# TangJiakai/RecBole-FairRec

Hardware: AMD Instinct MI355X
Metric: training interactions/sec + achieved HBM GB/s, FOCF emb=64 at 1/2/4/8 MI355X (higher is better)
Workload: dtype f32; 1 GPU; FOCF fair_objective=value, 1000001 users x 100001 items, embedding_size=64, B=8192 per GPU, Adam lr=1e-3 weight_decay=1e-3 (BASELINE.json configs[1]); ranks_seen=1, item_distribution=uniform, launch=hipGraph, lazy_adam_sweep_period=123, tables=single GPU, global_batch=8192, aged_steps=123

## Files before the change

### recbole-fairrec_amd/csrc/focf_step.hip

```cpp
#include <stddef.h>
#include <stdlib.h>

#include <algorithm>

#include "common.hpp"
#include "kernels.hpp"
#include "table.hpp"
#include "focf_ws.hpp"
#include "focf_loss.hpp"

namespace fr {

#ifndef FR_LPT_SHARED_FIRST
#define FR_LPT_SHARED_FIRST 1
#endif
#ifndef FR_STEP_WPB
#define FR_STEP_WPB 4
#endif
constexpr int STEP_WPB = FR_STEP_WPB;

struct StepArgs {
    float *Up, *Um, *Uv;
    int32_t *Ulast, *Ustamp;
    float *Ip, *Im, *Iv;
    int32_t *Ilast, *Istamp;
    int D, step;
    AdamC c;
    int B, objective;
    float fair_weight;
    const int4* task_rec;
    const int4* task_info;
    int lead;
    const int32_t* hdr;
    float* mse_e;
    float* term;
    void* ws;
    long long lo_u, lo_i;
    int n_u, n_i, skip_from;
    const int32_t* sw_order;
    uint32_t* err;
    unsigned long long *hcu, *hci;
    PrevLoss prev;
};

struct KV {
    unsigned v0, v1;
};
template <typename T>
__device__ __forceinline__ T karg(KV kv, int off) {
    static_assert(sizeof(T) == 4 || sizeof(T) == 8, "4- or 8-byte argument fields");
    const int d = off >> 2;
    auto word = [&](int i) { return (unsigned)__builtin_amdgcn_readlane((int)(i < 64 ? kv.v0 : kv.v1), i & 63); };
    if constexpr (sizeof(T) == 4) {
        return __builtin_bit_cast(T, word(d));
    } else {
        const unsigned long long q = (unsigned long long)word(d) | ((unsigned long long)word(d + 1) << 32);
        return __builtin_bit_cast(T, q);
    }
}
#define KA(field) karg<decltype(StepArgs::field)>(kv, (int)offsetof(StepArgs, field))
#define KAC(field) karg<decltype(AdamC::field)>(kv, (int)(offsetof(StepArgs, c) + offsetof(AdamC, field)))
static_assert(sizeof(StepArgs) <= 512, "the argument block must fit two VGPRs of dwords");

__device__ __forceinline__ int4 uload4(const int4* p, int idx) {
    const int4 v = p[idx];
    return make_int4(uniform(v.x), uniform(v.y), uniform(v.z), uniform(v.w));
}
__device__ __forceinline__ int uload(const int32_t* p, long long idx) { return uniform(p[idx]); }

__device__ __forceinline__ float ld_sc1(const float* p) {
    return __hip_atomic_load(p, __ATOMIC_RELAXED, __HIP_MEMORY_SCOPE_AGENT);
}
__device__ __forceinline__ void st_sc1(float* p, float v) {
    __hip_atomic_store(p, v, __ATOMIC_RELAXED, __HIP_MEMORY_SCOPE_AGENT);
}
__device__ __forceinline__ void drain_stores() { asm volatile("s_waitcnt vmcnt(0)" ::: "memory"); }

typedef __attribute__((address_space(1))) float gfloat;
typedef __attribute__((address_space(1))) int32_t gint;
__device__ __forceinline__ const gfloat* gp(const float* p) { return (const gfloat*)p; }
__device__ __forceinline__ gfloat* gp(float* p) { return (gfloat*)p; }
__device__ __forceinline__ const gint* gp(const int32_t* p) { return (const gint*)p; }
__device__ __forceinline__ gint* gp(int32_t* p) { return (gint*)p; }
typedef int v4i_ __attribute__((ext_vector_type(4)));
typedef __attribute__((address_space(1))) v4i_ gint4;
struct GInt4Ptr {
    const gint4* p;
    __device__ __forceinline__ int4 operator[](long long i) const {
        const v4i_ v = p[i];
        return make_int4(v.x, v.y, v.z, v.w);
    }
};
__device__ __forceinline__ GInt4Ptr gp(const int4* p) { return GInt4Ptr{(const gint4*)p}; }

__device__ __forceinline__ void st_sc1g(gfloat* p, float v) {
    __hip_atomic_store(p, v, __ATOMIC_RELAXED, __HIP_MEMORY_SCOPE_AGENT);
}

template <int E, bool FULL>
__device__ __forceinline__ void ldrow(RowFrag<E>& f, const float* base, int D, int lane) {
    const gfloat* g = gp(base);
#pragma unroll
    for (int e = 0; e < E; ++e) {
        const int d = lane + 64 * e;
        f.x[e] = (FULL || d < D) ? g[d] : 0.f;
    }
}

template <int E, bool FULL>
__device__ __forceinline__ void load_row_sc1(RowFrag<E>& f, const float* base, int D, int lane) {
    const gfloat* g = gp(base);
#pragma unroll
    for (int e = 0; e < E; ++e) {
        const int d = lane + 64 * e;
        f.x[e] = (FULL || d < D) ? __hip_atomic_load(g + d, __ATOMIC_RELAXED, __HIP_MEMORY_SCOPE_AGENT) : 0.f;
    }
}

template <int E, bool FULL>
__device__ __forceinline__ void store_row_sc1(const RowFrag<E>& f, float* base, int D, int lane) {
    gfloat* g = gp(base);
#pragma unroll
    for (int e = 0; e < E; ++e) {
        const int d = lane + 64 * e;
        float val = f.x[e];
        asm volatile("" : "+v"(val));
        if (FULL || d < D) st_sc1g(g + d, val);
    }
}

#ifndef FR_TROW_STORE
#define FR_TROW_STORE 1
#endif
#ifndef FR_WORD_STORE
#define FR_WORD_STORE 1
#endif
__device__ __forceinline__ void store_word(int32_t* p, int v) {
#if FR_TROW_STORE == 1 && FR_WORD_STORE
    __hip_atomic_store((gint*)p, v, __ATOMIC_RELAXED, __HIP_MEMORY_SCOPE_AGENT);
#else
    *(gint*)p = v;
#endif
}
__device__ __forceinline__ void store_word(float* p, float v) {
#if FR_TROW_STORE == 1 && FR_WORD_STORE
    st_sc1g((gfloat*)p, v);
#else
    *(gfloat*)p = v;
#endif
}

template <int E, bool FULL, bool WT = true>
__device__ __forceinline__ void store_trow(const RowFrag<E>& f, float* base, int D, int lane) {
    gfloat* g = gp(base);
#pragma unroll
    for (int e = 0; e < E; ++e) {
        const int d = lane + 64 * e;
#if FR_TROW_STORE == 1
        if (WT) {
            if (FULL || d < D) { float val = f.x[e]; asm volatile("" : "+v"(val)); st_sc1g(g + d, val); }
        } else if (FULL || d < D) g[d] = f.x[e];
#elif FR_TROW_STORE == 2
        if (WT) {
            if (FULL || d < D) __builtin_nontemporal_store(f.x[e], g + d);
        } else if (FULL || d < D) g[d] = f.x[e];
#else
        if (FULL || d < D) g[d] = f.x[e];
#endif
    }
}

constexpr int SW_NC = 16;
constexpr int HC_TAG_SHIFT = 29;
constexpr unsigned long long HC_CNT1 = 1ull << 14;
__device__ __forceinline__ int hc_base(unsigned long long w) { return (int)(w & 0x3fffull); }
__device__ __forceinline__ int hc_cnt(unsigned long long w) { return (int)((w >> 14) & 0x7fffull); }
static_assert(FR_SORT_MAX <= (1 << 14), "a batch's member list is addressed with 14 bits");

__device__ __forceinline__ unsigned ord_enc(float x) {
    const unsigned b = __float_as_uint(x);
    return (b & 0x80000000u) ? ~b : (b | 0x80000000u);
}
__device__ __forceinline__ float ord_dec(unsigned e) { return __uint_as_float((e & 0x80000000u) ? (e & 0x7fffffffu) : ~e); }

struct ClaimJob {
    const int64_t *user, *item;
    const float *rating, *sst;
    int4 *rec, *info;
    int32_t* cp;
    unsigned long long *hcu, *hci;
    int B, stamp;
    long long lo_u, lo_i;
    int n_u, n_i;
    int32_t* sw_tmp;
};
struct PlaceJob {
    int4 *rec, *info, *task_rec, *task_info;
    int32_t *cp, *hdr;
    unsigned long long *hcu, *hci;
    int B, n_pairs, stamp;
    const int32_t* sw_tmp;
    int32_t* sw_order;
};
struct StageArgs {
    ClaimJob c;
    PlaceJob p;
    int nb_claim, nb_sa, nb_place, nb_sb;
    int32_t *Ulast, *Ustamp, *Ilast, *Istamp;
    int n_rows_u, n_rows_i, cap;
    uint32_t* err;
};
constexpr int STAGE_THREADS = 64 * STEP_WPB;

template <int NC>
__device__ __forceinline__ int class_rank(int k, int32_t* counters, int lane) {
    const unsigned long long lt = (1ull << lane) - 1ull;
    unsigned long long m[NC];
    int mine = 0;
#pragma unroll
    for (int c = 0; c < NC; ++c) {
        m[c] = __ballot(k == c);
        if (lane == c) mine = __popcll(m[c]);
    }
    int got = 0;
    if (lane < NC && mine) got = atomicAdd(counters + lane, mine);
    int rk = 0;
#pragma unroll
    for (int c = 0; c < NC; ++c) {
        const int base = __shfl(got, c, 64);
        if (k == c) rk = base + __popcll(m[c] & lt);
    }
    return rk;
}

__device__ __forceinline__ int replay_class(int a, int b, int cap, int NC) {
    a = a < 0 ? 0 : (a > cap ? cap : a);
    b = b < 0 ? 0 : (b > cap ? cap : b);
    const int hi = a > b ? a : b, lo = a > b ? b : a;
    const int cost = 7 * hi + 2 * lo;
    return NC - 1 - min(NC - 1, cost * NC / (9 * cap + 1));
}

#ifndef FR_STAGE_EPT
#define FR_STAGE_EPT 2
#endif
constexpr int STAGE_EPT = FR_STAGE_EPT;
constexpr int STAGE_BLOCK = STAGE_THREADS * STAGE_EPT;

__device__ __forceinline__ void stage_claim(const StageArgs& s, int sb) {
    const ClaimJob& J = s.c;
    const int lane = threadIdx.x & 63;
    constexpr int EPT = STAGE_EPT;
    int b[EPT];
    bool ok[EPT];
    long long u[EPT], i[EPT];
    float rt[EPT], ss[EPT];
#pragma unroll
    for (int e = 0; e < EPT; ++e) {
        b[e] = (sb * EPT + e) * STAGE_THREADS + (int)threadIdx.x;
        ok[e] = b[e] < J.B;
        const int bc = ok[e] ? b[e] : 0;
        u[e] = J.user[bc];
        i[e] = J.item[bc];
        rt[e] = J.rating[bc];
        ss[e] = J.sst ? J.sst[bc] : 0.f;
    }
    bool bad = false;
#pragma unroll
    for (int e = 0; e < EPT; ++e) {
        bad |= ok[e] && (u[e] < 0 || u[e] >= s.n_rows_u || i[e] < 0 || i[e] >= s.n_rows_i);
        if (u[e] < 0 || u[e] >= s.n_rows_u) u[e] = 0;
        if (i[e] < 0 || i[e] >= s.n_rows_i) i[e] = 0;
    }
    if (bad && s.err) atomicOr(s.err, FR_DEV_ERR_INDEX_RANGE);
    const unsigned long long T = (unsigned long long)J.stamp << HC_TAG_SHIFT;
    unsigned long long mu[EPT], mi[EPT], ou[EPT], oi[EPT];
#pragma unroll
    for (int e = 0; e < EPT; ++e) {
        mu[e] = mi[e] = 0ull;
        if (ok[e]) {
            mu[e] = __hip_atomic_fetch_max(J.hcu + u[e], T, __ATOMIC_RELAXED, __HIP_MEMORY_SCOPE_AGENT);
            mi[e] = __hip_atomic_fetch_max(J.hci + i[e], T, __ATOMIC_RELAXED, __HIP_MEMORY_SCOPE_AGENT);
            atomicMax(s.Ustamp + u[e], J.stamp);
            atomicMax(s.Istamp + i[e], J.stamp);
        }
    }
#pragma unroll
    for (int e = 0; e < EPT; ++e) {
        ou[e] = oi[e] = 0ull;
        if (ok[e]) {
            ou[e] = __hip_atomic_fetch_add(J.hcu + u[e], HC_CNT1 + (mu[e] >> 63), __ATOMIC_RELAXED, __HIP_MEMORY_SCOPE_AGENT);
            oi[e] = __hip_atomic_fetch_add(J.hci + i[e], HC_CNT1 + (mi[e] >> 63), __ATOMIC_RELAXED, __HIP_MEMORY_SCOPE_AGENT);
        }
    }
    int first = 0;
    unsigned e1 = 0u, e2 = 0u;
#pragma unroll
    for (int e = 0; e < EPT; ++e) {
        const int ru = hc_cnt(ou[e]), ri = hc_cnt(oi[e]);
        if (ok[e]) {
            J.rec[b[e]] = make_int4((int)u[e], (int)i[e], __float_as_int(rt[e]), __float_as_int(ss[e]));
            J.info[b[e]] = make_int4(ru, ri, 0, 0);
            e1 = max(e1, ord_enc(ss[e]));
            e2 = max(e2, ord_enc(-ss[e]));
        }
        first += __popcll(__ballot(ok[e] && ri == 0));
    }
    if (lane == 0 && first) atomicAdd(J.cp + 8, first);
    if (J.sst) {
#pragma unroll
        for (int o = 32; o > 0; o >>= 1) {
            e1 = max(e1, (unsigned)__shfl_xor((int)e1, o, 64));
            e2 = max(e2, (unsigned)__shfl_xor((int)e2, o, 64));
        }
        if (lane == 0) {
            atomicMax(reinterpret_cast<unsigned*>(J.cp + 9), e1);
            atomicMax(reinterpret_cast<unsigned*>(J.cp + 10), e2);
        }
    }
}

__device__ __forceinline__ void stage_sweep_class(const StageArgs& s, int sb) {
    const ClaimJob& J = s.c;
    const int lane = threadIdx.x & 63;
    constexpr int EPT = STAGE_EPT;
    const int pairs_u = (J.n_u + 1) >> 1, n_pairs = pairs_u + ((J.n_i + 1) >> 1);
    const int cap = s.cap > 0 ? s.cap : 1024;
    int q[EPT], la[EPT], lb[EPT], sa[EPT], sb_[EPT], k[EPT];
#pragma unroll
    for (int e = 0; e < EPT; ++e) {
        q[e] = (sb * EPT + e) * STAGE_THREADS + (int)threadIdx.x;
        const int qc = q[e] < n_pairs ? q[e] : 0;
        const bool inU = qc < pairs_u;
        const int kk = inU ? qc : qc - pairs_u;
        const long long rowA = (inU ? J.lo_u : J.lo_i) + 2 * kk;
        const long long rowB = 2 * kk + 1 < (inU ? J.n_u : J.n_i) ? rowA + 1 : rowA;
        const int32_t* Tl = inU ? s.Ulast : s.Ilast;
        const int32_t* Ts = inU ? s.Ustamp : s.Istamp;
        la[e] = Tl[rowA]; lb[e] = Tl[rowB]; sa[e] = Ts[rowA]; sb_[e] = Ts[rowB];
    }
    int mine = 0;
#pragma unroll
    for (int e = 0; e < EPT; ++e) {
        k[e] = q[e] < n_pairs ? replay_class(sa[e] >= J.stamp ? 0 : J.stamp - la[e], sb_[e] >= J.stamp ? 0 : J.stamp - lb[e],
                                            cap, SW_NC)
                              : -1;
#pragma unroll
        for (int c = 0; c < SW_NC; ++c) {
            const int n = __popcll(__ballot(k[e] == c));
            if (lane == c) mine += n;
        }
    }
    int got = 0;
    if (lane < SW_NC && mine) got = atomicAdd(J.cp + 16 + lane, mine);
    const unsigned long long lt = (1ull << lane) - 1ull;
    int rk[EPT];
#pragma unroll
    for (int e = 0; e < EPT; ++e) rk[e] = 0;
#pragma unroll
    for (int c = 0; c < SW_NC; ++c) {
        int run = __shfl(got, c, 64);
#pragma unroll
        for (int e = 0; e < EPT; ++e) {
            const unsigned long long m = __ballot(k[e] == c);
            if (k[e] == c) rk[e] = run + __popcll(m & lt);
            run += __popcll(m);
        }
    }
#pragma unroll
    for (int e = 0; e < EPT; ++e)
        if (k[e] >= 0) J.sw_tmp[q[e]] = k[e] << 20 | rk[e];
}

#ifndef FR_PLACE_EPT
#define FR_PLACE_EPT 1
#endif
constexpr int PLACE_EPT = FR_PLACE_EPT;
__device__ __forceinline__ void stage_place(const StageArgs& s, int sb) {
    const PlaceJob& J = s.p;
    const int lane = threadIdx.x & 63;
    constexpr int EPT = PLACE_EPT;
    int b[EPT];
    bool ok[EPT];
    int4 rec[EPT], f[EPT];
#pragma unroll
    for (int e = 0; e < EPT; ++e) {
        b[e] = (sb * EPT + e) * STAGE_THREADS + (int)threadIdx.x;
        ok[e] = b[e] < J.B;
        const int bc = ok[e] ? b[e] : 0;
        rec[e] = J.rec[bc];
        f[e] = J.info[bc];
    }
    int nu[EPT], ni[EPT], k[EPT], key[EPT];
    {
        unsigned long long wu[EPT], wi[EPT];
        int lu[EPT], li[EPT];
#pragma unroll
        for (int e = 0; e < EPT; ++e) {
            wu[e] = J.hcu[rec[e].x];
            wi[e] = J.hci[rec[e].y];
            lu[e] = s.Ulast[rec[e].x];
            li[e] = s.Ilast[rec[e].y];
        }
        const int cap = s.cap > 0 ? s.cap : 1024;
#pragma unroll
        for (int e = 0; e < EPT; ++e) {
            nu[e] = hc_cnt(wu[e]);
            ni[e] = hc_cnt(wi[e]);
            if (ok[e] && nu[e] > 1 && f[e].x == 0) {
                const int base = atomicAdd(J.cp + 11, nu[e]);
                __hip_atomic_fetch_add(J.hcu + rec[e].x, (unsigned long long)base, __ATOMIC_RELAXED, __HIP_MEMORY_SCOPE_AGENT);
            }
            if (ok[e] && ni[e] > 1 && f[e].y == 0) {
                const int base = atomicAdd(J.cp + 12, ni[e]);
                __hip_atomic_fetch_add(J.hci + rec[e].y, (unsigned long long)base, __ATOMIC_RELAXED, __HIP_MEMORY_SCOPE_AGENT);
            }
            k[e] = !ok[e] ? -1 : ((nu[e] > 1 || ni[e] > 1) && FR_LPT_SHARED_FIRST ? 0 : 1);
            int cu = J.stamp - 1 - lu[e], ci = J.stamp - 1 - li[e];
            cu = cu < 0 ? 0 : (cu > cap ? cap : cu);
            ci = ci < 0 ? 0 : (ci > cap ? cap : ci);
            key[e] = 7 * (cu > ci ? cu : ci) + 2 * (cu > ci ? ci : cu);
        }
    }
    int before[EPT];
#pragma unroll
    for (int e = 0; e < EPT; ++e) before[e] = 0;
    int n0 = 0, n1 = 0;
#pragma unroll
    for (int e2 = 0; e2 < EPT; ++e2) {
        n0 += __popcll(__ballot(k[e2] == 0));
        n1 += __popcll(__ballot(k[e2] == 1));
        for (int t = 0; t < 64; ++t) {
            const int kt = __builtin_amdgcn_readlane(k[e2], t), ct = __builtin_amdgcn_readlane(key[e2], t);
#pragma unroll
            for (int e = 0; e < EPT; ++e)
                before[e] += (kt == k[e] && (ct > key[e] || (ct == key[e] && (e2 < e || (e2 == e && t < lane))))) ? 1 : 0;
        }
    }
    int got = 0;
    if (lane == 0 && n0) got = atomicAdd(J.cp, n0);
    if (lane == 1 && n1) got = atomicAdd(J.cp + 1, n1);
    const int base0 = __shfl(got, 0, 64), base1 = __shfl(got, 1, 64);
#pragma unroll
    for (int e = 0; e < EPT; ++e) {
        if (!ok[e]) continue;
        const int pos = k[e] == 0 ? base0 + before[e] : J.B - 1 - (base1 + (n1 - 1 - before[e]));
        J.task_rec[pos] = rec[e];
        J.task_info[pos] = make_int4(f[e].x | nu[e] << 16, f[e].y | ni[e] << 16, 0, b[e]);
        J.info[b[e]] = make_int4(f[e].x, f[e].y, nu[e], ni[e]);
    }
    if (sb == 0 && threadIdx.x == 0) {
        const unsigned e1 = (unsigned)J.cp[9], e2 = (unsigned)J.cp[10];
        *reinterpret_cast<int4*>(J.hdr) = make_int4(J.cp[8], 0, __float_as_int(-ord_dec(e2)), __float_as_int(ord_dec(e1)));
    }
}

__device__ __forceinline__ void stage_sweep_place(const StageArgs& s, int sb) {
    const PlaceJob& J = s.p;
    int cnt[SW_NC];
#pragma unroll
    for (int c = 0; c < SW_NC; ++c) cnt[c] = J.cp[16 + c];
    int v[STAGE_EPT];
#pragma unroll
    for (int e = 0; e < STAGE_EPT; ++e) {
        const int q = (sb * STAGE_EPT + e) * STAGE_THREADS + (int)threadIdx.x;
        v[e] = q < J.n_pairs ? J.sw_tmp[q] : -1;
    }
#pragma unroll
    for (int e = 0; e < STAGE_EPT; ++e) {
        const int q = (sb * STAGE_EPT + e) * STAGE_THREADS + (int)threadIdx.x;
        if (v[e] >= 0) {
            const int k = v[e] >> 20;
            int pos = v[e] & 0xfffff;
#pragma unroll
            for (int c = 0; c < SW_NC; ++c) pos += c < k ? cnt[c] : 0;
            J.sw_order[pos] = q;
        }
    }
    if (sb == 0 && threadIdx.x == 0) J.sw_order[J.n_pairs] = J.n_pairs;
}

__device__ __forceinline__ void stage_block(const StageArgs& s, int sb) {
    if (sb < s.nb_claim) return stage_claim(s, sb);
    sb -= s.nb_claim;
    if (sb < s.nb_sa) return stage_sweep_class(s, sb);
    sb -= s.nb_sa;
    if (sb < s.nb_place) return stage_place(s, sb);
    sb -= s.nb_place;
    if (sb < s.nb_sb) stage_sweep_place(s, sb);
}

__device__ __forceinline__ unsigned long long uniform64(unsigned long long x) {
    return (unsigned long long)(unsigned)uniform((int)(unsigned)x) | ((unsigned long long)(unsigned)uniform((int)(x >> 32)) << 32);
}
__device__ __forceinline__ int ld_sc1_int(const int32_t* p) {
    return __hip_atomic_load(p, __ATOMIC_RELAXED, __HIP_MEMORY_SCOPE_AGENT);
}
__device__ __forceinline__ void st_sc1_int(int32_t* p, int v) {
    __hip_atomic_store(p, v, __ATOMIC_RELAXED, __HIP_MEMORY_SCOPE_AGENT);
}
__device__ __forceinline__ unsigned long long hc_arrive(unsigned long long* p, int lane) {
    unsigned long long t = 0;
    if (lane == 0) t = __hip_atomic_fetch_add(p, 0ull - HC_CNT1, __ATOMIC_RELAXED, __HIP_MEMORY_SCOPE_AGENT);
    return uniform64(t);
}

struct Members {
    int reg;
    const int32_t* sorted;
    int n;
};
__device__ __forceinline__ Members load_members(const int32_t* list, int32_t* sorted, int base, int n, int lane) {
    Members m;
    m.n = n;
    m.reg = 0;
    m.sorted = sorted + base;
    if (n <= 64) {
        const int v = lane < n ? ld_sc1_int(list + base + lane) : 0x7fffffff;
        int rank = 0;
        for (int t = 0; t < n; ++t) rank += __builtin_amdgcn_readlane(v, t) < v ? 1 : 0;
        m.reg = __builtin_amdgcn_ds_permute(rank << 2, v);
        return m;
    }
    for (int jb = 0; jb < n; jb += 64) {
        const int v = jb + lane < n ? ld_sc1_int(list + base + jb + lane) : 0x7fffffff;
        int rank = 0;
        for (int jc = 0; jc < n; jc += 64) {
            const int x = jc + lane < n ? ld_sc1_int(list + base + jc + lane) : 0x7fffffff;
            const int cn = min(64, n - jc);
            for (int t = 0; t < cn; ++t) rank += __builtin_amdgcn_readlane(x, t) < v ? 1 : 0;
        }
        if (jb + lane < n) st_sc1_int(sorted + base + rank, v);
    }
    drain_stores();
    return m;
}
__device__ __forceinline__ int members_chunk(const Members& m, int jb, int lane) {
    if (m.n <= 64) return lane < m.n ? m.reg : 0;
    int idx = jb + lane;
    asm volatile("" : "+v"(idx));
    return idx < m.n ? ld_sc1_int(m.sorted + idx) : 0;
}

__device__ __forceinline__ bool arrive_last(unsigned int* cnt, int n, int lane) {
    unsigned t = 0;
    if (lane == 0) t = __hip_atomic_fetch_add(cnt, 1u, __ATOMIC_RELAXED, __HIP_MEMORY_SCOPE_AGENT);
    t = (unsigned)uniform((int)t);
    if (t != (unsigned)(n - 1)) return false;
    if (lane == 0) *cnt = 0u;
    return true;
}

template <int E, bool FULL>
__device__ __forceinline__ void adam_write(float* Tp, float* Tm, float* Tv, int32_t* Tlast, int D, int step,
                                           const AdamC& c, int row, RowFrag<E>& p, RowFrag<E>& m, RowFrag<E>& v,
                                           const RowFrag<E>& g, float2 s, int lane) {
#pragma unroll
    for (int e = 0; e < E; ++e) adam_elem(p.x[e], m.x[e], v.x[e], g.x[e], s.x, s.y, c);
    store_trow<E, FULL, false>(p, Tp + (size_t)row * D, D, lane);
    store_trow<E, FULL, false>(m, Tm + (size_t)row * D, D, lane);
    store_trow<E, FULL, false>(v, Tv + (size_t)row * D, D, lane);
    if (lane == 0) Tlast[row] = step;
}

template <int E, bool FULL, typename Chunk>
__device__ __forceinline__ void handed_grad_sum(RowFrag<E>& g, int n, Chunk chunk, const float* coef, const float* other,
                                                int D, int lane) {
#pragma unroll
    for (int e = 0; e < E; ++e) g.x[e] = 0.f;
    constexpr int UN = 2;
    for (int jb = 0; jb < n; jb += 64) {
        const int cnt = min(64, n - jb);
        int my_b = chunk(jb);
        float my_c = 0.f;
        if (lane >= cnt) my_b = 0;
        if (lane < cnt) my_c = ld_sc1(coef + my_b);
        for (int t0 = 0; t0 < cnt; t0 += UN) {
            RowFrag<E> o[UN];
            float cb[UN];
#pragma unroll
            for (int q = 0; q < UN; ++q) {
                const int t = t0 + q < cnt ? t0 + q : cnt - 1;
                const int b = __builtin_amdgcn_readlane(my_b, t);
                cb[q] = __builtin_bit_cast(float, __builtin_amdgcn_readlane(__builtin_bit_cast(int, my_c), t));
                load_row_sc1<E, FULL>(o[q], other + (size_t)b * D, D, lane);
            }
            {
#pragma clang fp contract(off)
#pragma unroll
                for (int q = 0; q < UN; ++q) {
                    if (t0 + q < cnt) {
#pragma unroll
                        for (int e = 0; e < E; ++e) {
                            float prod = cb[q] * o[q].x[e];
                            g.x[e] = g.x[e] + prod;
                        }
                    }
                }
            }
        }
    }
}

template <int E>
struct TwoRows {
    RowFrag<E> pA, mA, vA, pB, mB, vB;
};

template <int E>
__device__ __forceinline__ TwoRows<E> replay_two_v(TwoRows<E> r, int tA, int tB, int upto, const AdamC& c, int lane) {
    tA = tA < upto ? tA : upto;
    tB = tB < upto ? tB : upto;
    if (tA != tB) {
        const bool a_old = tA < tB;
        RowFrag<E> p, m, v;
#pragma unroll
        for (int e = 0; e < E; ++e) {
            p.x[e] = a_old ? r.pA.x[e] : r.pB.x[e];
            m.x[e] = a_old ? r.mA.x[e] : r.mB.x[e];
            v.x[e] = a_old ? r.vA.x[e] : r.vB.x[e];
        }
        replay<E>(p, m, v, a_old ? tA : tB, a_old ? tB : tA, c, lane);
#pragma unroll
        for (int e = 0; e < E; ++e) {
            if (a_old) {
                r.pA.x[e] = p.x[e]; r.mA.x[e] = m.x[e]; r.vA.x[e] = v.x[e];
            } else {
                r.pB.x[e] = p.x[e]; r.mB.x[e] = m.x[e]; r.vB.x[e] = v.x[e];
            }
        }
    }
    replay2<E>(r.pA, r.mA, r.vA, r.pB, r.mB, r.vB, tA > tB ? tA : tB, upto, c, lane);
    return r;
}
template <int E>
__device__ __forceinline__ void replay_two(TwoRows<E>& r, int tA, int tB, int upto, const AdamC& c, int lane) {
    r = replay_two_v<E>(r, tA, tB, upto, c, lane);
}

template <int E, bool FULL>
__device__ __forceinline__ void user_finish(KV kv, const AdamC& c, const FocfWs& w, int j0u, int nu, float2 s, int lane) {
    const int D = FULL ? 64 * E : KA(D);
    const int c0 = uniform(w.perm_u[j0u]);
    const int ur = uniform(w.rec[c0].x);
    RowFrag<E> p, m, v, g;
    load_row_sc1<E, FULL>(p, w.side[0] + (size_t)c0 * D, D, lane);
    load_row_sc1<E, FULL>(m, w.side[1] + (size_t)c0 * D, D, lane);
    load_row_sc1<E, FULL>(v, w.side[2] + (size_t)c0 * D, D, lane);
    handed_grad_sum<E, FULL>(g, nu, [&](int jb) { return jb + lane < nu ? w.perm_u[j0u + jb + lane] : 0; }, w.coef, w.side[3],
                             D, lane);
    adam_write<E, FULL>(KA(Up), KA(Um), KA(Uv), KA(Ulast), D, KA(step), c, ur, p, m, v, g, s, lane);
}

template <int E, bool FULL>
__device__ __forceinline__ void user_finish_c(KV kv, const AdamC& c, const FocfWs& w, int ur, int base, int nu, float2 s,
                                              int lane) {
    const int D = FULL ? 64 * E : KA(D);
    const Members mem = load_members(w.perm_u, w.seg_start_u, base, nu, lane);
    const int c0 = __builtin_amdgcn_readlane(members_chunk(mem, 0, lane), 0);
    RowFrag<E> p, m, v, g;
    load_row_sc1<E, FULL>(p, w.side[0] + (size_t)c0 * D, D, lane);
    load_row_sc1<E, FULL>(m, w.side[1] + (size_t)c0 * D, D, lane);
    load_row_sc1<E, FULL>(v, w.side[2] + (size_t)c0 * D, D, lane);
    handed_grad_sum<E, FULL>(g, nu, [&](int jb) { return members_chunk(mem, jb, lane); }, w.coef, w.side[3], D, lane);
    adam_write<E, FULL>(KA(Up), KA(Um), KA(Uv), KA(Ulast), D, KA(step), c, ur, p, m, v, g, s, lane);
}

template <int E, bool FULL, bool CLAIM>
__device__ __forceinline__ void step_shared_rows(KV kv, const AdamC& c, int b, int lane, int ur, int ir, int iux, int iix,
                                                 int seg_u, int seg_i, float dot, float coef, float smin, float smax,
                                                 float K, RowFrag<E>& pu, RowFrag<E>& mu, RowFrag<E>& vu, RowFrag<E>& pi,
                                                 RowFrag<E>& mi, RowFrag<E>& vi) {
    const int D = FULL ? 64 * E : KA(D);
    const bool fair = KA(objective) != FR_FOCF_NONE;
    const int nu = iux >> 16, ni = iix >> 16, j0u = iux & 0xffff, j0i = iix & 0xffff;
    const float2 s = step_scalars(c, KA(step));
    int Bq = KA(B);
    asm volatile("" : "+s"(Bq));
    const FocfWs w = focf_layout(KA(ws), Bq, D);

    if constexpr (CLAIM) {
        unsigned long long wu = 0, wi = 0;
        if (nu > 1) wu = __hip_atomic_load(KA(hcu) + ur, __ATOMIC_RELAXED, __HIP_MEMORY_SCOPE_AGENT);
        if (ni > 1) wi = __hip_atomic_load(KA(hci) + ir, __ATOMIC_RELAXED, __HIP_MEMORY_SCOPE_AGENT);
        if (lane == 0) {
            if (nu > 1) st_sc1_int(w.perm_u + hc_base(wu) + j0u, b);
            if (ni > 1) st_sc1_int(w.perm_i + hc_base(wi) + j0i, b);
        }
    }
    const size_t so = (size_t)b * D;
    store_row_sc1<E, FULL>(pu, w.side[0] + so, D, lane);
    store_row_sc1<E, FULL>(mu, w.side[1] + so, D, lane);
    store_row_sc1<E, FULL>(vu, w.side[2] + so, D, lane);
    if (nu > 1) store_row_sc1<E, FULL>(pi, w.side[3] + so, D, lane);
    if (ni == 1) {
        RowFrag<E> gi;
#pragma unroll
        for (int e = 0; e < E; ++e) gi.x[e] = coef * pu.x[e];
        adam_write<E, FULL>(KA(Ip), KA(Im), KA(Iv), KA(Ilast), D, KA(step), c, ir, pi, mi, vi, gi, s, lane);
        if (lane == 0) st_sc1(w.coef + b, coef);
        drain_stores();
        if constexpr (CLAIM) {
            const unsigned long long old = hc_arrive(KA(hcu) + ur, lane);
            if (hc_cnt(old) == 1) user_finish_c<E, FULL>(kv, c, w, ur, hc_base(old), nu, s, lane);
        } else {
            if (arrive_last(w.cnt_u + seg_u, nu, lane)) user_finish<E, FULL>(kv, c, w, j0u, nu, s, lane);
        }
        return;
    }
    if (lane == 0) {
        st_sc1(w.pred + b, dot);
        if (CLAIM && fair) st_sc1(w.term + b, 0.f);
    }
    drain_stores();
    Members mem{};
    if constexpr (CLAIM) {
        const unsigned long long old = hc_arrive(KA(hci) + ir, lane);
        if (hc_cnt(old) != 1) return;
        mem = load_members(w.perm_i, w.seg_start_i, hc_base(old), ni, lane);
    } else {
        if (!arrive_last(w.cnt_i + seg_i, ni, lane)) return;
    }

    const bool big = ni > 64;
    int my_b = 0, my_u = 0, my_iux = 0, my_seg = 0;
    float my_pr = 0.f, my_rt = 0.f, my_s = 0.f;
    auto load_chunk = [&](int jb) {
        my_b = 0; my_u = 0; my_iux = 0; my_seg = 0;
        my_pr = 0.f; my_rt = 0.f; my_s = 0.f;
        int mb = 0;
        if constexpr (CLAIM) mb = members_chunk(mem, jb, lane);
        if (jb + lane < ni) {
            if constexpr (CLAIM) my_b = mb;
            else my_b = w.perm_i[j0i + jb + lane];
            const int4 rq = w.rec[my_b];
            const int4 fq = w.info[my_b];
            my_pr = ld_sc1(w.pred + my_b);
            my_u = rq.x; my_rt = __int_as_float(rq.z); my_s = __int_as_float(rq.w);
            if constexpr (CLAIM) {
                my_iux = fq.z << 16;
            } else {
                my_iux = fq.x; my_seg = fq.y;
            }
        }
    };
    float term = 0.f, g0 = 0.f, g1 = 0.f;
    if (fair) {
        float sp0 = 0.f, sp1 = 0.f, st0 = 0.f, st1 = 0.f, n0 = 0.f, n1 = 0.f;
        bool bad = false;
        int first_b = 0;
        for (int jb = 0; jb < ni; jb += 64) {
            load_chunk(jb);
            if (jb == 0) first_b = __builtin_amdgcn_readlane(my_b, 0);
#pragma unroll
            for (int k = 0; k < 64 / FAIR_GROUP; ++k) {
                const int src = (lane & (FAIR_GROUP - 1)) + FAIR_GROUP * k;
                const float pr = __shfl(my_pr, src, 64), rr = __shfl(my_rt, src, 64), sq = __shfl(my_s, src, 64);
                if (lane < FAIR_GROUP && jb + src < ni) {
                    bad |= (sq != smin && sq != smax);
                    if (sq == smin) {
                        sp0 += pr; st0 += rr; n0 += 1.f;
                    } else {
                        sp1 += pr; st1 += rr; n1 += 1.f;
                    }
                }
            }
        }
        if (bad && KA(err)) atomicOr(KA(err), FR_DEV_ERR_SST_GROUPS);
        sp0 = group_sum<FAIR_GROUP>(sp0); sp1 = group_sum<FAIR_GROUP>(sp1);
        st0 = group_sum<FAIR_GROUP>(st0); st1 = group_sum<FAIR_GROUP>(st1);
        n0 = group_sum<FAIR_GROUP>(n0);   n1 = group_sum<FAIR_GROUP>(n1);
        sp0 = __builtin_bit_cast(float, uniform(__builtin_bit_cast(int, sp0)));
        sp1 = __builtin_bit_cast(float, uniform(__builtin_bit_cast(int, sp1)));
        st0 = __builtin_bit_cast(float, uniform(__builtin_bit_cast(int, st0)));
        st1 = __builtin_bit_cast(float, uniform(__builtin_bit_cast(int, st1)));
        n0 = __builtin_bit_cast(float, uniform(__builtin_bit_cast(int, n0)));
        n1 = __builtin_bit_cast(float, uniform(__builtin_bit_cast(int, n1)));
        focf_fair_eval(KA(objective), KA(fair_weight), K, sp0, sp1, st0, st1, n0, n1, term, g0, g1);
        if (lane == 0) KA(term)[CLAIM ? first_b : seg_i] = term;
    }
    constexpr int UN = E == 1 ? 4 : (E == 2 ? 2 : 1);
    RowFrag<E> gi;
#pragma unroll
    for (int e = 0; e < E; ++e) gi.x[e] = 0.f;
    bool shared_users = false;
    for (int jb = 0; jb < ni; jb += 64) {
        if (big || !fair) load_chunk(jb);
        const int cnt = min(64, ni - jb);
        float my_c = 0.f;
        if (lane < cnt) {
            const float erq = my_pr - my_rt;
            my_c = 2.f * erq / (float)KA(B);
            if (fair) my_c = my_c + (my_s == smin ? g0 : g1);
            if ((my_iux >> 16) > 1) st_sc1(w.coef + my_b, my_c);
        }
        shared_users |= __ballot(lane < cnt && (my_iux >> 16) > 1) != 0ull;
        for (int t0 = 0; t0 < cnt; t0 += UN) {
            RowFrag<E> p[UN], m[UN], v[UN];
            int uq[UN], nq[UN];
            float cq[UN];
#pragma unroll
            for (int q = 0; q < UN; ++q) {
                const int t = t0 + q < cnt ? t0 + q : cnt - 1;
                const int bq = __builtin_amdgcn_readlane(my_b, t);
                uq[q] = __builtin_amdgcn_readlane(my_u, t);
                nq[q] = __builtin_amdgcn_readlane(my_iux, t) >> 16;
                cq[q] = __builtin_bit_cast(float, __builtin_amdgcn_readlane(__builtin_bit_cast(int, my_c), t));
                const size_t sq = (size_t)bq * D;
                load_row_sc1<E, FULL>(p[q], w.side[0] + sq, D, lane);
                load_row_sc1<E, FULL>(m[q], w.side[1] + sq, D, lane);
                load_row_sc1<E, FULL>(v[q], w.side[2] + sq, D, lane);
            }
#pragma unroll
            for (int q = 0; q < UN; ++q) {
                if (t0 + q >= cnt) continue;
                {
#pragma clang fp contract(off)
#pragma unroll
                    for (int e = 0; e < E; ++e) {
                        float prod = cq[q] * p[q].x[e];
                        gi.x[e] = gi.x[e] + prod;
                    }
                }
                if (nq[q] == 1) {
                    RowFrag<E> gu;
#pragma unroll
                    for (int e = 0; e < E; ++e) gu.x[e] = cq[q] * pi.x[e];
                    adam_write<E, FULL>(KA(Up), KA(Um), KA(Uv), KA(Ulast), D, KA(step), c, uq[q], p[q], m[q], v[q], gu, s, lane);
                }
            }
        }
    }
    adam_write<E, FULL>(KA(Ip), KA(Im), KA(Iv), KA(Ilast), D, KA(step), c, ir, pi, mi, vi, gi, s, lane);
    if (!shared_users) return;
    drain_stores();
    for (int jb = 0; jb < ni; jb += 64) {
        if (big) load_chunk(jb);
        const int cnt = min(64, ni - jb);
        unsigned long long todo = __ballot(lane < cnt && (my_iux >> 16) > 1);
        while (todo) {
            const int t = __builtin_ctzll(todo);
            todo &= todo - 1;
            const int iq = __builtin_amdgcn_readlane(my_iux, t);
            if constexpr (CLAIM) {
                const int uu = __builtin_amdgcn_readlane(my_u, t);
                const unsigned long long old = hc_arrive(KA(hcu) + uu, lane);
                if (hc_cnt(old) == 1) user_finish_c<E, FULL>(kv, c, w, uu, hc_base(old), iq >> 16, s, lane);
            } else {
                const int sg = __builtin_amdgcn_readlane(my_seg, t);
                if (arrive_last(w.cnt_u + sg, iq >> 16, lane)) user_finish<E, FULL>(kv, c, w, iq & 0xffff, iq >> 16, s, lane);
            }
        }
    }
}

__device__ __forceinline__ void focf_fair_single(int objective, float fair_weight, float K, bool in0, float pred,
                                                 float rating, float& term, float& g) {
    const float cc = 1.f + 1e-5f;
    const float P = pred / cc, T = rating / cc;
    float d, q;
    if (objective == FR_FOCF_VALUE) {
        d = P - T; q = 1.f;
    } else if (objective == FR_FOCF_ABSOLUTE) {
        d = fabsf(P - T); q = (P > T) ? 1.f : (P < T ? -1.f : 0.f);
    } else if (objective == FR_FOCF_UNDER) {
        d = (T - P > 0.f) ? T - P : 0.f; q = (T - P > 0.f) ? -1.f : 0.f;
    } else {
        d = (P - T > 0.f) ? P - T : 0.f; q = (P - T > 0.f) ? 1.f : 0.f;
    }
    const float delta = in0 ? d - 0.f : 0.f - d;
    const float x = fabsf(delta);
    term = smooth_l1(x);
    const float sgn = delta > 0.f ? 1.f : (delta < 0.f ? -1.f : 0.f);
    const float dx = (x < 1.f ? x : 1.f) * sgn * fair_weight / K;
    g = in0 ? dx * q / cc : -dx * q / cc;
}

template <int E, bool FULL, bool CLAIM>
__device__ __forceinline__ void step_finish(KV kv, const AdamC& c, int lane, int q, RowFrag<E>& pu, RowFrag<E>& mu,
                                            RowFrag<E>& vu, RowFrag<E>& pi, RowFrag<E>& mi, RowFrag<E>& vi) {
    const int D = FULL ? 64 * E : KA(D);
    const bool fair = KA(objective) != FR_FOCF_NONE;
    const int4 vrec = KA(task_rec)[q], vinf = KA(task_info)[q], vhd = *reinterpret_cast<const int4*>(KA(hdr));
    const int4 rec = make_int4(uniform(vrec.x), uniform(vrec.y), uniform(vrec.z), uniform(vrec.w));
    const int4 inf = make_int4(uniform(vinf.x), uniform(vinf.y), uniform(vinf.z), uniform(vinf.w));
    const int4 hd = make_int4(uniform(vhd.x), 0, uniform(vhd.z), uniform(vhd.w));
    const int ur = rec.x, ir = rec.y;
    const float rt = __int_as_float(rec.z), s = __int_as_float(rec.w);
    const int iux = inf.x, iix = inf.y, b = inf.w;
    const float K = (float)hd.x, smin = __int_as_float(hd.z), smax = __int_as_float(hd.w);
    const int nu = iux >> 16, ni = iix >> 16, seg_u = inf.z & 0xffff, seg_i = inf.z >> 16;
    float dot = 0.f;
#pragma unroll
    for (int e = 0; e < E; ++e) dot = fmaf(pu.x[e], pi.x[e], dot);
    dot = wave_sum(dot);
    const float er = dot - rt;
    if (lane == 0) store_word(KA(mse_e) + b, er * er);
    const float cm = 2.f * er / (float)KA(B);
    float coef = cm;
    if (ni == 1 && fair) {
        const bool in0 = s == smin;
        if (s != smin && s != smax && lane == 0 && KA(err)) atomicOr(KA(err), FR_DEV_ERR_SST_GROUPS);
        float term, g;
        focf_fair_single(KA(objective), KA(fair_weight), K, in0, dot, rt, term, g);
        coef = cm + g;
        if (lane == 0) KA(term)[CLAIM ? b : seg_i] = term;
    }
    if (ni == 1 && nu == 1) {
        const float2 sc = step_scalars(c, KA(step));
#pragma unroll
        for (int e = 0; e < E; ++e) {
            v2f_ P = {pu.x[e], pi.x[e]}, M = {mu.x[e], mi.x[e]}, V = {vu.x[e], vi.x[e]};
            const v2f_ G = __builtin_elementwise_fma(v2f_{c.wd, c.wd}, P, v2f_{coef * P.y, coef * P.x});
            M = __builtin_elementwise_fma(v2f_{c.omb1, c.omb1}, G - M, M);
            V = __builtin_elementwise_fma(G * c.omb2, G, V * c.b2);
            const v2f_ den = __builtin_elementwise_fma(v2f_{__builtin_amdgcn_sqrtf(V.x), __builtin_amdgcn_sqrtf(V.y)},
                                                      v2f_{sc.y, sc.y}, v2f_{c.eps, c.eps});
            P = __builtin_elementwise_fma(M * -sc.x, v2f_{__builtin_amdgcn_rcpf(den.x), __builtin_amdgcn_rcpf(den.y)}, P);
            pu.x[e] = P.x; pi.x[e] = P.y;
            mu.x[e] = M.x; mi.x[e] = M.y;
            vu.x[e] = V.x; vi.x[e] = V.y;
        }
        store_trow<E, FULL>(pu, KA(Up) + (size_t)ur * D, D, lane);
        store_trow<E, FULL>(mu, KA(Um) + (size_t)ur * D, D, lane);
        store_trow<E, FULL>(vu, KA(Uv) + (size_t)ur * D, D, lane);
        store_trow<E, FULL>(pi, KA(Ip) + (size_t)ir * D, D, lane);
        store_trow<E, FULL>(mi, KA(Im) + (size_t)ir * D, D, lane);
        store_trow<E, FULL>(vi, KA(Iv) + (size_t)ir * D, D, lane);
        if (lane == 0) {
            store_word(KA(Ulast) + ur, KA(step));
            store_word(KA(Ilast) + ir, KA(step));
        }
        return;
    }
    step_shared_rows<E, FULL, CLAIM>(kv, c, b, lane, ur, ir, iux, iix, seg_u, seg_i, dot, coef, smin, smax, K, pu, mu, vu, pi, mi,
                                     vi);
}

template <int E, bool FULL>
__device__ __forceinline__ void adam_store_both(KV kv, const AdamC& c, int lane, int ur, int ir, float coef, float2 sc,
                                                RowFrag<E> pu, RowFrag<E> mu, RowFrag<E> vu, RowFrag<E> pi,
                                                RowFrag<E> mi, RowFrag<E> vi) {
    const int D = FULL ? 64 * E : KA(D);
#pragma unroll
    for (int e = 0; e < E; ++e) {
        v2f_ P = {pu.x[e], pi.x[e]}, M = {mu.x[e], mi.x[e]}, V = {vu.x[e], vi.x[e]};
        const v2f_ G = __builtin_elementwise_fma(v2f_{c.wd, c.wd}, P, v2f_{coef * P.y, coef * P.x});
        M = __builtin_elementwise_fma(v2f_{c.omb1, c.omb1}, G - M, M);
        V = __builtin_elementwise_fma(G * c.omb2, G, V * c.b2);
        const v2f_ den = __builtin_elementwise_fma(v2f_{__builtin_amdgcn_sqrtf(V.x), __builtin_amdgcn_sqrtf(V.y)},
                                                  v2f_{sc.y, sc.y}, v2f_{c.eps, c.eps});
        P = __builtin_elementwise_fma(M * -sc.x, v2f_{__builtin_amdgcn_rcpf(den.x), __builtin_amdgcn_rcpf(den.y)}, P);
        pu.x[e] = P.x; pi.x[e] = P.y;
        mu.x[e] = M.x; mi.x[e] = M.y;
        vu.x[e] = V.x; vi.x[e] = V.y;
    }
    store_trow<E, FULL>(pu, KA(Up) + (size_t)ur * D, D, lane);
    store_trow<E, FULL>(mu, KA(Um) + (size_t)ur * D, D, lane);
    store_trow<E, FULL>(vu, KA(Uv) + (size_t)ur * D, D, lane);
    store_trow<E, FULL>(pi, KA(Ip) + (size_t)ir * D, D, lane);
    store_trow<E, FULL>(mi, KA(Im) + (size_t)ir * D, D, lane);
    store_trow<E, FULL>(vi, KA(Iv) + (size_t)ir * D, D, lane);
    if (lane == 0) {
        store_word(KA(Ulast) + ur, KA(step));
        store_word(KA(Ilast) + ir, KA(step));
    }
}

template <int E, bool FULL, bool CLAIM>
__device__ __forceinline__ void step_finish_pair(KV kv, const AdamC& c, int lane, int q, int q1, bool has1, TwoRows<E> us,
                                                 TwoRows<E> is) {
    const int obj = KA(objective);
    const bool fair = obj != FR_FOCF_NONE;
    const GInt4Ptr trec = gp(KA(task_rec));
    const GInt4Ptr tinf = gp(KA(task_info));
    const int4 vr0 = trec[q], vr1 = trec[q1], vi0 = tinf[q], vi1 = tinf[q1];
    const int4 vhd = gp(reinterpret_cast<const int4*>(KA(hdr)))[0];
    float d0 = 0.f, d1 = 0.f;
#pragma unroll
    for (int e = 0; e < E; ++e) {
        d0 = fmaf(us.pA.x[e], is.pA.x[e], d0);
        d1 = fmaf(us.pB.x[e], is.pB.x[e], d1);
    }
#pragma unroll
    for (int o = 32; o > 0; o >>= 1) {
        const float y0 = __shfl_xor(d0, o, 64), y1 = __shfl_xor(d1, o, 64);
        d0 += y0;
        d1 += y1;
    }
    const bool odd = (lane & 1) != 0;
    const int rec_z = odd ? vr1.z : vr0.z, rec_w = odd ? vr1.w : vr0.w;
    const int inf_y = odd ? vi1.y : vi0.y, inf_z = odd ? vi1.z : vi0.z, inf_w = odd ? vi1.w : vi0.w;
    const float dot = odd ? d1 : d0;
    const float rt = __int_as_float(rec_z), sst = __int_as_float(rec_w);
    const float K = (float)vhd.x, smin = __int_as_float(vhd.z), smax = __int_as_float(vhd.w);
    const int ni_l = inf_y >> 16;
    const float er = dot - rt;
    const float cm = 2.f * er / (float)KA(B);
    float coef = cm, term = 0.f;
    const bool single = fair && ni_l == 1;
    if (fair) {
        float g;
        focf_fair_single(obj, KA(fair_weight), K, sst == smin, dot, rt, term, g);
        if (single) coef = cm + g;
    }
    if (lane < (has1 ? 2 : 1)) {
        store_word(KA(mse_e) + inf_w, er * er);
        if (single) {
            store_word(KA(term) + (CLAIM ? inf_w : inf_z >> 16), term);
            if (sst != smin && sst != smax && KA(err)) atomicOr(KA(err), FR_DEV_ERR_SST_GROUPS);
        }
    }
    const float coef0 = __builtin_bit_cast(float, __builtin_amdgcn_readlane(__builtin_bit_cast(int, coef), 0));
    const float coef1 = __builtin_bit_cast(float, __builtin_amdgcn_readlane(__builtin_bit_cast(int, coef), 1));
    const int ur0 = uniform(vr0.x), ir0 = uniform(vr0.y), ur1 = uniform(vr1.x), ir1 = uniform(vr1.y);
    const int iux0 = uniform(vi0.x), iix0 = uniform(vi0.y), iux1 = uniform(vi1.x), iix1 = uniform(vi1.y);
    const bool un0 = (iux0 >> 16) == 1 && (iix0 >> 16) == 1;
    const bool un1 = has1 && (iux1 >> 16) == 1 && (iix1 >> 16) == 1;
    const float2 sc = step_scalars(c, KA(step));
    if (un0 && un1) {
        RowFrag<E> a0 = us.pA, a1 = us.mA, a2 = us.vA, a3 = is.pA, a4 = is.mA, a5 = is.vA;
        RowFrag<E> b0 = us.pB, b1 = us.mB, b2 = us.vB, b3 = is.pB, b4 = is.mB, b5 = is.vB;
        adam_store_both<E, FULL>(kv, c, lane, ur0, ir0, coef0, sc, a0, a1, a2, a3, a4, a5);
        adam_store_both<E, FULL>(kv, c, lane, ur1, ir1, coef1, sc, b0, b1, b2, b3, b4, b5);
        return;
    }
    if (un0) adam_store_both<E, FULL>(kv, c, lane, ur0, ir0, coef0, sc, us.pA, us.mA, us.vA, is.pA, is.mA, is.vA);
    if (un1) adam_store_both<E, FULL>(kv, c, lane, ur1, ir1, coef1, sc, us.pB, us.mB, us.vB, is.pB, is.mB, is.vB);
    if (un0 && (un1 || !has1)) return;
    for (int k = 0; k < (has1 ? 2 : 1); ++k) {
        if (k) {
#pragma unroll
            for (int e = 0; e < E; ++e) {
                us.pA.x[e] = us.pB.x[e]; us.mA.x[e] = us.mB.x[e]; us.vA.x[e] = us.vB.x[e];
                is.pA.x[e] = is.pB.x[e]; is.mA.x[e] = is.mB.x[e]; is.vA.x[e] = is.vB.x[e];
            }
        }
        if (!(k ? un1 : un0)) {
            const int sg = uniform(k ? vi1.z : vi0.z);
            step_shared_rows<E, FULL, CLAIM>(kv, c, uniform(k ? vi1.w : vi0.w), lane, k ? ur1 : ur0, k ? ir1 : ir0, k ? iux1 : iux0,
                                      k ? iix1 : iix0, sg & 0xffff, sg >> 16, k ? d1 : d0, k ? coef1 : coef0, smin, smax, K,
                                      us.pA, us.mA, us.vA, is.pA, is.mA, is.vA);
        }
    }
}

#if FR_STEP_TRACE
#define g_phase phase_stamps
#endif
template <int E, bool FULL, bool PAIR, bool CLAIM>
__device__ __forceinline__ void step_task(KV kv, bool sweeper, int q, int n_pairs, int lane, const int4* rec0,
                                          const int32_t* order0, int B0
#if FR_STEP_TRACE
                                          , unsigned long long (&phase_stamps)[4]
#endif
) {
    asm volatile("" : "+v"(lane));
    AdamC c;
    c.sc = KAC(sc); c.cap = KAC(cap); c.wd = KAC(wd); c.b1 = KAC(b1); c.omb1 = KAC(omb1); c.b2 = KAC(b2); c.omb2 = KAC(omb2);
    c.eps = KAC(eps); c.k1 = KAC(k1); c.k2 = KAC(k2); c.inv_k1 = KAC(inv_k1); c.inv_k2 = KAC(inv_k2);
    const int D = FULL ? 64 * E : KA(D);
    TwoRows<E> r;
    int tA, tB;
    if (sweeper) {
        if (const int32_t* so = order0) {
            const int oq = so[q], on = so[n_pairs];
            q = uniform(on) == n_pairs ? uniform(oq) : q;
        }
        const int pairs_u = (KA(n_u) + 1) >> 1;
        const bool inU = q < pairs_u;
        const int k = inU ? q : q - pairs_u;
        const long long rowA = (inU ? KA(lo_u) : KA(lo_i)) + 2 * k;
        const bool hasB = 2 * k + 1 < (inU ? KA(n_u) : KA(n_i));
        const long long rowB = hasB ? rowA + 1 : rowA;
        float* Tp = inU ? KA(Up) : KA(Ip);
        float* Tm = inU ? KA(Um) : KA(Im);
        float* Tv = inU ? KA(Uv) : KA(Iv);
        int32_t* Tl = inU ? KA(Ulast) : KA(Ilast);
        const int32_t* Ts = inU ? KA(Ustamp) : KA(Istamp);
        const int sa = gp(Ts)[rowA], sb = gp(Ts)[rowB];
        const int la = gp((const int32_t*)Tl)[rowA], lb = gp((const int32_t*)Tl)[rowB];
        ldrow<E, FULL>(r.pA, Tp + (size_t)rowA * D, D, lane);
        ldrow<E, FULL>(r.mA, Tm + (size_t)rowA * D, D, lane);
        ldrow<E, FULL>(r.vA, Tv + (size_t)rowA * D, D, lane);
        ldrow<E, FULL>(r.pB, Tp + (size_t)rowB * D, D, lane);
        ldrow<E, FULL>(r.mB, Tm + (size_t)rowB * D, D, lane);
        ldrow<E, FULL>(r.vB, Tv + (size_t)rowB * D, D, lane);
        const int upto = KA(step);
        tA = uniform(sa) >= KA(skip_from) ? upto : uniform(la);
        tB = (!hasB || uniform(sb) >= KA(skip_from)) ? upto : uniform(lb);
        const bool doA = tA < upto, doB = tB < upto;
        replay_two<E>(r, tA, tB, upto, c, lane);
        if (doA) {
            store_trow<E, FULL>(r.pA, Tp + (size_t)rowA * D, D, lane);
            store_trow<E, FULL>(r.mA, Tm + (size_t)rowA * D, D, lane);
            store_trow<E, FULL>(r.vA, Tv + (size_t)rowA * D, D, lane);
            if (lane == 0) store_word(Tl + rowA, upto);
        }
        if (doB) {
            store_trow<E, FULL>(r.pB, Tp + (size_t)rowB * D, D, lane);
            store_trow<E, FULL>(r.mB, Tm + (size_t)rowB * D, D, lane);
            store_trow<E, FULL>(r.vB, Tv + (size_t)rowB * D, D, lane);
            if (lane == 0) store_word(Tl + rowB, upto);
        }
        return;
    }
    if (PAIR) {
        const bool has1 = q + 1 < B0;
        const int q1 = has1 ? q + 1 : q;
        const int4 vrec0 = gp(rec0)[q], vrec1 = gp(rec0)[q1];
        const int u0 = uniform(vrec0.x), i0 = uniform(vrec0.y), u1 = uniform(vrec1.x), i1 = uniform(vrec1.y);
#if FR_STEP_TRACE
        g_phase[2] = __builtin_amdgcn_s_memrealtime();
#endif
        const int lu0 = gp((const int32_t*)KA(Ulast))[u0], lu1 = gp((const int32_t*)KA(Ulast))[u1];
        const int li0 = gp((const int32_t*)KA(Ilast))[i0], li1 = gp((const int32_t*)KA(Ilast))[i1];
        TwoRows<E> it;
        ldrow<E, FULL>(r.pA, KA(Up) + (size_t)u0 * D, D, lane);
        ldrow<E, FULL>(r.pB, KA(Up) + (size_t)u1 * D, D, lane);
        ldrow<E, FULL>(it.pA, KA(Ip) + (size_t)i0 * D, D, lane);
        ldrow<E, FULL>(it.pB, KA(Ip) + (size_t)i1 * D, D, lane);
        ldrow<E, FULL>(r.mA, KA(Um) + (size_t)u0 * D, D, lane);
        ldrow<E, FULL>(r.vA, KA(Uv) + (size_t)u0 * D, D, lane);
        ldrow<E, FULL>(r.mB, KA(Um) + (size_t)u1 * D, D, lane);
        ldrow<E, FULL>(r.vB, KA(Uv) + (size_t)u1 * D, D, lane);
        ldrow<E, FULL>(it.mA, KA(Im) + (size_t)i0 * D, D, lane);
        ldrow<E, FULL>(it.vA, KA(Iv) + (size_t)i0 * D, D, lane);
        ldrow<E, FULL>(it.mB, KA(Im) + (size_t)i1 * D, D, lane);
        ldrow<E, FULL>(it.vB, KA(Iv) + (size_t)i1 * D, D, lane);
        const int upto = KA(step) - 1;
        const int tu0 = uniform(lu0), tu1 = uniform(lu1), ti0 = uniform(li0), ti1 = uniform(li1);
#if FR_STEP_TRACE
        g_phase[0] = __builtin_amdgcn_s_memrealtime();
        g_phase[3] = (unsigned long long)((upto - tu0) + (upto - tu1) + (upto - ti0) + (upto - ti1));
#endif
        replay_two<E>(r, tu0, tu1, upto, c, lane);
        replay_two<E>(it, ti0, ti1, upto, c, lane);
#if FR_STEP_TRACE
        g_phase[1] = __builtin_amdgcn_s_memrealtime();
#endif
        step_finish_pair<E, FULL, CLAIM>(kv, c, lane, q, q1, has1, r, it);
        return;
    }
    const int4 vrec = rec0[q];
    const int ur = uniform(vrec.x), ir = uniform(vrec.y);
    const int lu = KA(Ulast)[ur], li = KA(Ilast)[ir];
    ldrow<E, FULL>(r.pA, KA(Up) + (size_t)ur * D, D, lane);
    ldrow<E, FULL>(r.pB, KA(Ip) + (size_t)ir * D, D, lane);
    ldrow<E, FULL>(r.mA, KA(Um) + (size_t)ur * D, D, lane);
    ldrow<E, FULL>(r.vA, KA(Uv) + (size_t)ur * D, D, lane);
    ldrow<E, FULL>(r.mB, KA(Im) + (size_t)ir * D, D, lane);
    ldrow<E, FULL>(r.vB, KA(Iv) + (size_t)ir * D, D, lane);
    tA = uniform(lu);
    tB = uniform(li);
    replay_two<E>(r, tA, tB, KA(step) - 1, c, lane);
    step_finish<E, FULL, CLAIM>(kv, c, lane, q, r.pA, r.mA, r.vA, r.pB, r.mB, r.vB);
}

__host__ __device__ constexpr bool step_pairs(int E) { return E <= 1; }

#ifndef FR_STEP_TRACE
#define FR_STEP_TRACE 0
#endif

#if FR_STEP_TRACE
__device__ unsigned long long g_step_trace[8 * 65536];
__device__ int g_trace_step = -1;
#endif

#ifndef FR_STEP_WAVES
#define FR_STEP_WAVES 6
#endif
__host__ __device__ constexpr int step_waves(int E) { return E >= 4 ? (FR_STEP_WAVES < 5 ? FR_STEP_WAVES : 5) : FR_STEP_WAVES; }
constexpr int STEP_PRELOAD_DWORDS = 10;
template <int E, bool FULL, bool CLAIM>
__global__ __launch_bounds__(64 * STEP_WPB, step_waves(E)) void focf_step_kernel(const int4* pre_rec, const int32_t* pre_order,
                                                                                 int pre_B, int pre_lead, int pre_nu, int pre_ni,
                                                                                 int pre_stage, int pre_pad, StepArgs a,
                                                                                 StageArgs st) {
#if FR_STEP_TRACE
    const unsigned long long tr0 = __builtin_amdgcn_s_memrealtime();
    const unsigned long long mt0 = __builtin_amdgcn_s_memtime();
    unsigned long long ph[4] = {0, 0, 0, 0};
#endif
    const int lane = threadIdx.x & 63;
    const int wib = uniform((int)(threadIdx.x >> 6));
    int role = 0;
    const int n_stage = CLAIM ? pre_stage : 0;
    (void)pre_pad;
#ifndef FR_STAGE_POS
#define FR_STAGE_POS 2
#endif
    const int stage0 = FR_STAGE_POS == 0 ? 1 : (FR_STAGE_POS == 1 ? (int)gridDim.x - n_stage : 1 + pre_lead);
    if (blockIdx.x == 0) {
        if (a.prev.loss_out) step_reduce_loss<64 * STEP_WPB>(a.prev);
    } else if (CLAIM && (int)blockIdx.x >= stage0 && (int)blockIdx.x < stage0 + n_stage) {
        if constexpr (CLAIM) stage_block(st, (int)blockIdx.x - stage0);
        role = 3;
    } else {
        const unsigned* kp = reinterpret_cast<const unsigned*>(
            (const void*)(const __attribute__((address_space(4))) void*)__builtin_amdgcn_kernarg_segment_ptr());
        KV kv;
        static_assert(STEP_PRELOAD_DWORDS * 4 % alignof(StepArgs) == 0, "StepArgs follows the preloaded scalars without padding");
        kv.v0 = kp[STEP_PRELOAD_DWORDS + lane];
        kv.v1 = lane < (int)(sizeof(StepArgs) / 4) - 64 ? kp[STEP_PRELOAD_DWORDS + 64 + lane] : 0u;
        const int x = (int)blockIdx.x - 1 - ((int)blockIdx.x >= stage0 ? n_stage : 0);
        const int n_pairs = ((pre_nu + 1) >> 1) + ((pre_ni + 1) >> 1);
        const int n_sweep = n_pairs;
        const int ns = (n_sweep + STEP_WPB - 1) / STEP_WPB;
        constexpr bool PAIR = step_pairs(E);
        const bool sweeper = x >= pre_lead && x < pre_lead + ns;
        const int q = ((sweeper ? x - pre_lead : (x < pre_lead ? x : x - ns)) * STEP_WPB + wib) * (!sweeper && PAIR ? 2 : 1);
        role = sweeper ? 1 : 2;
#if FR_STEP_TRACE
        if (q < (sweeper ? n_sweep : pre_B)) step_task<E, FULL, PAIR, CLAIM>(kv, sweeper, q, n_pairs, lane, pre_rec, pre_order, pre_B, ph);
#else
        if (q < (sweeper ? n_sweep : pre_B)) step_task<E, FULL, PAIR, CLAIM>(kv, sweeper, q, n_pairs, lane, pre_rec, pre_order, pre_B);
#endif
    }
#if FR_STEP_TRACE
    asm volatile("s_waitcnt vmcnt(0)" ::: "memory");
    const unsigned long long tr1 = __builtin_amdgcn_s_memrealtime();
    const unsigned long long mt1 = __builtin_amdgcn_s_memtime();
    unsigned hw, xcc;
    asm volatile("s_getreg_b32 %0, hwreg(HW_REG_HW_ID)" : "=s"(hw));
    asm volatile("s_getreg_b32 %0, hwreg(HW_REG_XCC_ID)" : "=s"(xcc));
    const int tsel = g_trace_step < 0 ? 0 : a.step - g_trace_step;
    const unsigned wq = blockIdx.x * STEP_WPB + wib + (g_trace_step < 0 ? 0u : 16384u * (unsigned)(tsel & 3));
    if (lane == 0 && wq < 65536 && (g_trace_step < 0 || (tsel >= 0 && tsel < 4 && blockIdx.x * STEP_WPB + wib < 16384))) {
        g_step_trace[4 * wq] = tr0;
        g_step_trace[4 * wq + 1] = tr1;
        g_step_trace[4 * wq + 2] = role;
        g_step_trace[4 * wq + 3] = (unsigned long long)hw | ((unsigned long long)xcc << 32);
        g_step_trace[4 * (65536 + wq)] = (ph[2] ? ((ph[2] - tr0) << 40) : 0ull) | (mt1 - mt0);
        g_step_trace[4 * (65536 + wq) + 1] = ph[0];
        g_step_trace[4 * (65536 + wq) + 2] = ph[1];
        g_step_trace[4 * (65536 + wq) + 3] = ph[3];
    }
#endif
}

__global__ __launch_bounds__(256) void focf_step_finish_kernel(PrevLoss pl) { step_reduce_loss<256>(pl); }

__global__ __launch_bounds__(STAGE_THREADS) void focf_stage_kernel(StageArgs st) { stage_block(st, (int)blockIdx.x); }

struct SwOrderJob {
    const int32_t *Ulast, *Ustamp, *Ilast, *Istamp;
    long long lo_u, lo_i;
    int n_u, n_i, upto, skip_from;
    int32_t* order;
};

template <int PT>
__device__ __forceinline__ void sweep_order_body(const SwOrderJob& J, int cap_, int* cnt, int* wsum) {
    constexpr int NC = SW_NC, NW = 16, N = NC * PT * NW, EPT = (N + 1023) / 1024;
    const int tid = threadIdx.x, lane = tid & 63, wave = tid >> 6;
    const unsigned long long lt = (1ull << lane) - 1ull;
    const int cap = cap_ > 0 ? cap_ : 1024;
    const int pairs_u = (J.n_u + 1) >> 1, n_pairs = pairs_u + ((J.n_i + 1) >> 1);
    if (!J.order) return;
    if (n_pairs > PT * 1024) {
        if (tid == 0 && n_pairs <= SWEEP_ORDER_MAX) J.order[n_pairs] = -1;
        return;
    }
    int la[PT], lb[PT], sa[PT], sb[PT];
#pragma unroll
    for (int r = 0; r < PT; ++r) {
        const int q = r * 1024 + tid, qc = q < n_pairs ? q : 0;
        const bool inU = qc < pairs_u;
        const int k = inU ? qc : qc - pairs_u;
        const long long rowA = (inU ? J.lo_u : J.lo_i) + 2 * k;
        const long long rowB = 2 * k + 1 < (inU ? J.n_u : J.n_i) ? rowA + 1 : rowA;
        const int32_t* Tl = inU ? J.Ulast : J.Ilast;
        const int32_t* Ts = inU ? J.Ustamp : J.Istamp;
        la[r] = Tl[rowA]; lb[r] = Tl[rowB]; sa[r] = Ts[rowA]; sb[r] = Ts[rowB];
    }
    int cls[PT], rank[PT];
#pragma unroll
    for (int r = 0; r < PT; ++r) {
        const int q = r * 1024 + tid;
        int k = -1;
        if (q < n_pairs) {
            int ca = sa[r] >= J.skip_from ? 0 : J.upto - la[r], cb = sb[r] >= J.skip_from ? 0 : J.upto - lb[r];
            ca = ca < 0 ? 0 : (ca > cap ? cap : ca);
            cb = cb < 0 ? 0 : (cb > cap ? cap : cb);
            const int hi = ca > cb ? ca : cb, lo = ca > cb ? cb : ca;
            const int cost = 7 * hi + 2 * lo;
            k = NC - 1 - min(NC - 1, cost * NC / (9 * cap + 1));
        }
        cls[r] = k;
        rank[r] = 0;
#pragma unroll
        for (int c = 0; c < NC; ++c) {
            const unsigned long long m = __ballot(k == c);
            if (k == c) rank[r] = __popcll(m & lt);
            if (lane == 0) cnt[(c * PT + r) * NW + wave] = __popcll(m);
        }
    }
    __syncthreads();
    {
        int x[EPT], own = 0;
#pragma unroll
        for (int e = 0; e < EPT; ++e) {
            const int i = tid * EPT + e;
            x[e] = i < N ? cnt[i] : 0;
            own += x[e];
        }
        int inc = own;
#pragma unroll
        for (int o = 1; o < 64; o <<= 1) {
            const int y = __shfl_up(inc, o, 64);
            if (lane >= o) inc += y;
        }
        if (lane == 63) wsum[wave] = inc;
        __syncthreads();
        int ex = inc - own;
        for (int w = 0; w < wave; ++w) ex += wsum[w];
#pragma unroll
        for (int e = 0; e < EPT; ++e) {
            const int i = tid * EPT + e;
            if (i < N) cnt[i] = ex;
            ex += x[e];
        }
    }
    __syncthreads();
#pragma unroll
    for (int r = 0; r < PT; ++r)
        if (cls[r] >= 0) J.order[cnt[(cls[r] * PT + r) * NW + wave] + rank[r]] = r * 1024 + tid;
    if (tid == 0) J.order[n_pairs] = n_pairs;
}

struct LptJob {
    const int32_t *age_u, *age_i;
    const int4 *rec, *info;
    int4 *task_rec, *task_info;
    int B, upto;
};
struct LptJobs {
    LptJob j[FR_FOCF_PREPARE_MAX];
    SwOrderJob sw[FR_FOCF_PREPARE_MAX];
    int n;
    int cap;
};

#ifdef FR_LPT_STAMPS
__device__ unsigned long long g_lpt_stamps[8];
#define LPT_STAMP(i) do { if (blockIdx.x == 0 && threadIdx.x == 0) g_lpt_stamps[i] = __builtin_amdgcn_s_memtime(); } while (0)
#else
#define LPT_STAMP(i) do {} while (0)
#endif

constexpr int LPT_SPLIT = 4;

template <int PT>
__global__ __launch_bounds__(1024) void focf_lpt_kernel(LptJobs jobs) {
    constexpr int NC = 8, NW = 16, N = NC * PT * NW, EPT = (N + 1023) / 1024;
    __shared__ int cnt[SW_NC * PT * NW];
    __shared__ int wsum[NW];
    if ((int)blockIdx.x >= jobs.n * LPT_SPLIT) {
        sweep_order_body<PT>(jobs.sw[blockIdx.x - jobs.n * LPT_SPLIT], jobs.cap, cnt, wsum);
        return;
    }
    const LptJob& J = jobs.j[blockIdx.x / LPT_SPLIT];
    const int part = blockIdx.x % LPT_SPLIT;
    const int tid = threadIdx.x, lane = tid & 63, wave = tid >> 6;
    const unsigned long long lt = (1ull << lane) - 1ull;
    const int cap = jobs.cap > 0 ? jobs.cap : 1024;
    int cls[PT], rank[PT];
    int lu[PT], li[PT];
    bool sh[PT];
    LPT_STAMP(0);
#pragma unroll
    for (int q = 0; q < PT; ++q) {
        const int b = q * 1024 + tid, bc = b < J.B ? b : 0;
        lu[q] = J.age_u[bc];
        li[q] = J.age_i[bc];
#if FR_LPT_SHARED_FIRST
        const int4 f = J.info[bc];
        sh[q] = (f.x >> 16) > 1 || (f.z >> 16) > 1;
#else
        sh[q] = false;
#endif
    }
    LPT_STAMP(1);
#pragma unroll
    for (int q = 0; q < PT; ++q) {
        const int b = q * 1024 + tid;
        int k = -1;
        if (b < J.B) {
            int cu = J.upto - lu[q], ci = J.upto - li[q];
            cu = cu < 0 ? 0 : (cu > cap ? cap : cu);
            ci = ci < 0 ? 0 : (ci > cap ? cap : ci);
            const int hi = cu > ci ? cu : ci, lo = cu > ci ? ci : cu;
            const int cost = 7 * hi + 2 * lo;
            k = NC - 1 - min(NC - 1, cost * NC / (9 * cap + 1));
            if (sh[q]) k = 0;
        }
        cls[q] = k;
        rank[q] = 0;
#pragma unroll
        for (int c = 0; c < NC; ++c) {
            const unsigned long long m = __ballot(k == c);
            if (k == c) rank[q] = __popcll(m & lt);
            if (lane == 0) cnt[(c * PT + q) * NW + wave] = __popcll(m);
        }
    }
    LPT_STAMP(2);
    __syncthreads();
    {
        int x[EPT], own = 0;
#pragma unroll
        for (int e = 0; e < EPT; ++e) {
            const int i = tid * EPT + e;
            x[e] = i < N ? cnt[i] : 0;
            own += x[e];
        }
        int inc = own;
#pragma unroll
        for (int o = 1; o < 64; o <<= 1) {
            const int y = __shfl_up(inc, o, 64);
            if (lane >= o) inc += y;
        }
        if (lane == 63) wsum[wave] = inc;
        __syncthreads();
        int ex = inc - own;
        for (int w = 0; w < wave; ++w) ex += wsum[w];
#pragma unroll
        for (int e = 0; e < EPT; ++e) {
            const int i = tid * EPT + e;
            if (i < N) cnt[i] = ex;
            ex += x[e];
        }
    }
    __syncthreads();
    LPT_STAMP(3);
    constexpr int CH = (PT + LPT_SPLIT - 1) / LPT_SPLIT;
    int4 f[CH], r[CH];
#pragma unroll
    for (int q = 0; q < CH; ++q) {
        const int b = (q * LPT_SPLIT + part) * 1024 + tid, bc = b < J.B ? b : 0;
        f[q] = J.info[bc];
        r[q] = J.rec[bc];
    }
#pragma unroll
    for (int q = 0; q < CH; ++q) {
#pragma unroll
        for (int pp = 0; pp < LPT_SPLIT; ++pp) {
            const int qq = q * LPT_SPLIT + pp;
            if (pp == part && qq < PT && cls[qq] >= 0) {
                const int pos = cnt[(cls[qq] * PT + qq) * NW + wave] + rank[qq];
                J.task_rec[pos] = r[q];
                J.task_info[pos] = make_int4(f[q].x, f[q].z, f[q].y | (f[q].w << 16), qq * 1024 + tid);
            }
        }
    }
    LPT_STAMP(4);
}

}

using namespace fr;

extern "C" int fr_focf_prepare_step(const fr_focf_batch* batches, const int32_t* stamps, int32_t n, const fr_table* U,
                                    const fr_table* I, int32_t replay_cap, uint32_t* err_flag, void* stream_) {
    int rc;
    if ((rc = check_table(U, "fr_focf_prepare_step(U)")) || (rc = check_table(I, "fr_focf_prepare_step(I)"))) return rc;
    FR_CHECK_ARG(batches && stamps && n >= 1 && 2 * n <= FR_SORT_JOBS && U->dim == I->dim,
                 "fr_focf_prepare_step: 1..%d batches", FR_SORT_JOBS / 2);
    SortJobList jobs{};
    for (int q = 0; q < n; ++q) {
        const fr_focf_batch& b = batches[q];
        FR_CHECK_ARG(b.user && b.item && b.rating && b.ws && b.B >= 1 && b.B <= FR_SORT_MAX,
                     "fr_focf_prepare_step: batch %d", q);
        FocfWs w = focf_layout(b.ws, b.B, U->dim);
        FR_CHECK_ARG(b.ws_bytes >= w.bytes, "fr_focf_prepare_step: workspace %zu < %zu bytes", b.ws_bytes, w.bytes);
        SortJob ju{b.user, U->n_rows, w.perm_u, w.seg_start_u, w.seg_row_u, nullptr, w.nseg_u, nullptr, nullptr};
        SortJob ji{b.item, I->n_rows, w.perm_i, w.seg_start_i, w.seg_row_i, nullptr, w.nseg_i, b.sst, w.sst_minmax};
        ju.seg_first = w.seg_first_u;
        ji.seg_first = w.seg_first_i;
        ju.info = reinterpret_cast<int2*>(w.info);
        ji.info = reinterpret_cast<int2*>(w.info) + 1;
        ju.info_stride = ji.info_stride = 2;
        ji.rec = w.rec;
        ji.rec_idx = b.user;
        ji.rec_rows = U->n_rows;
        ji.rec_f0 = b.rating;
        ju.cnt = w.cnt_u;
        ji.cnt = w.cnt_i;
        ju.stamp = U->stamp;
        ji.stamp = I->stamp;
        ju.stamp_val = ji.stamp_val = stamps[q];
        ju.last = U->last;
        ji.last = I->last;
        ju.last_out = w.age_u;
        ji.last_out = w.age_i;
        ji.pos_of = w.pos_i;
        jobs.j[2 * q] = ju;
        jobs.j[2 * q + 1] = ji;
        jobs.M[2 * q] = jobs.M[2 * q + 1] = (int)b.B;
    }
    jobs.n = 2 * n;
    if ((rc = launch_sort_many(jobs, U->n_rows > I->n_rows ? U->n_rows : I->n_rows, err_flag, (hipStream_t)stream_)))
        return rc;
    LptJobs lj{};
    for (int q = 0; q < n; ++q) {
        const FocfWs w = focf_layout(batches[q].ws, batches[q].B, U->dim);
        lj.j[q] = LptJob{w.age_u, w.age_i, w.rec, w.info, w.task_rec, w.task_info, (int)batches[q].B, stamps[q] - 1};
    }
    lj.cap = replay_cap;
    lj.n = n;
    for (int q = 0; q < n; ++q) {
        const FocfWs w = focf_layout(batches[q].ws, batches[q].B, U->dim);
        fr_table tu = *U, ti = *I;
        tu.step = ti.step = stamps[q];
        const SweepSlice sw = make_sweep_slice(&tu, &ti, replay_cap);
        lj.sw[q] = SwOrderJob{U->last, U->stamp, I->last, I->stamp, sw.lo_u, sw.lo_i, sw.n_u, sw.n_i, stamps[q], stamps[q],
                              replay_cap > 0 ? w.sw_order : nullptr};
    }
    int Bmax = 1;
    for (int q = 0; q < n; ++q) Bmax = batches[q].B > Bmax ? (int)batches[q].B : Bmax;
    hipStream_t st = (hipStream_t)stream_;
    ProfScope prof(K_FOCF_LPT, st);
    if (Bmax <= 1024) FR_LAUNCH(prof, focf_lpt_kernel<1>, dim3(n * (LPT_SPLIT + 1)), dim3(1024), 0, st, lj);
    else if (Bmax <= 2048) FR_LAUNCH(prof, focf_lpt_kernel<2>, dim3(n * (LPT_SPLIT + 1)), dim3(1024), 0, st, lj);
    else if (Bmax <= 4096) FR_LAUNCH(prof, focf_lpt_kernel<4>, dim3(n * (LPT_SPLIT + 1)), dim3(1024), 0, st, lj);
    else if (Bmax <= 8192) FR_LAUNCH(prof, focf_lpt_kernel<8>, dim3(n * (LPT_SPLIT + 1)), dim3(1024), 0, st, lj);
    else FR_LAUNCH(prof, focf_lpt_kernel<16>, dim3(n * (LPT_SPLIT + 1)), dim3(1024), 0, st, lj);
    FR_CHECK_LAUNCH();
    return FR_OK;
}

static unsigned long long* words_of(uint64_t* row_words, int32_t gen, const fr_table* U, const fr_table* I, bool item) {
    const size_t per = (size_t)U->n_rows + (size_t)I->n_rows;
    return reinterpret_cast<unsigned long long*>(row_words) + (size_t)gen * per + (item ? (size_t)U->n_rows : 0);
}

static int make_stages(StageArgs& st, const fr_table* U, const fr_table* I, const fr_focf_batch* claim, int32_t claim_stamp,
                       int32_t claim_gen, const fr_focf_batch* place, int32_t place_stamp, int32_t place_gen,
                       int32_t sweep_period, uint64_t* row_words, uint32_t* err_flag, int32_t claim_step, int32_t place_step) {
    if (claim_step < 1) claim_step = claim_stamp;
    if (place_step < 1) place_step = place_stamp;
    st = StageArgs{};
    st.Ulast = U->last; st.Ustamp = U->stamp; st.Ilast = I->last; st.Istamp = I->stamp;
    st.n_rows_u = (int)U->n_rows; st.n_rows_i = (int)I->n_rows;
    st.cap = sweep_period;
    st.err = err_flag;
    FR_CHECK_ARG(row_words && U->n_rows <= INT32_MAX && I->n_rows <= INT32_MAX, "fr_focf_stage: row words missing");
    FR_CHECK_ARG(U->stamp && I->stamp && U->last && I->last, "fr_focf_stage: the tables need their last / stamp arrays");
    auto slice_of = [&](int32_t step) {
        fr_table tu = *U, ti = *I;
        tu.step = ti.step = step;
        return make_sweep_slice(&tu, &ti, sweep_period);
    };
    if (claim) {
        const fr_focf_batch& b = *claim;
        FR_CHECK_ARG(b.user && b.item && b.rating && b.ws && b.B >= 1 && b.B <= FR_SORT_MAX && claim_stamp >= 1 &&
                         claim_gen >= 0 && claim_gen < 3, "fr_focf_stage: batch to claim");
        const FocfWs w = focf_layout(b.ws, b.B, U->dim);
        FR_CHECK_ARG(b.ws_bytes >= w.bytes, "fr_focf_stage: workspace %zu < %zu bytes", b.ws_bytes, w.bytes);
        ClaimJob& J = st.c;
        J.user = b.user; J.item = b.item; J.rating = b.rating; J.sst = b.sst;
        J.rec = w.rec; J.info = w.info; J.cp = w.cp;
        J.hcu = words_of(row_words, claim_gen, U, I, false);
        J.hci = words_of(row_words, claim_gen, U, I, true);
        J.B = (int)b.B; J.stamp = claim_stamp;
        st.nb_claim = (int)((b.B + STAGE_BLOCK - 1) / STAGE_BLOCK);
        if (sweep_period > 0) {
            const SweepSlice sw = slice_of(claim_step);
            const long long n_pairs = ((long long)sw.n_u + 1) / 2 + ((long long)sw.n_i + 1) / 2;
            if (n_pairs <= SWEEP_ORDER_MAX) {
                J.lo_u = sw.lo_u; J.lo_i = sw.lo_i; J.n_u = sw.n_u; J.n_i = sw.n_i;
                J.sw_tmp = w.sw_tmp;
                st.nb_sa = (int)((n_pairs + STAGE_BLOCK - 1) / STAGE_BLOCK);
            }
        }
    }
    if (place) {
        const fr_focf_batch& b = *place;
        FR_CHECK_ARG(b.ws && b.B >= 1 && b.B <= FR_SORT_MAX && place_stamp >= 1 && place_gen >= 0 && place_gen < 3,
                     "fr_focf_stage: batch to place");
        const FocfWs w = focf_layout(b.ws, b.B, U->dim);
        FR_CHECK_ARG(b.ws_bytes >= w.bytes, "fr_focf_stage: workspace %zu < %zu bytes", b.ws_bytes, w.bytes);
        PlaceJob& J = st.p;
        J.rec = w.rec; J.info = w.info; J.task_rec = w.task_rec; J.task_info = w.task_info;
        J.cp = w.cp; J.hdr = w.nseg_i;
        J.hcu = words_of(row_words, place_gen, U, I, false);
        J.hci = words_of(row_words, place_gen, U, I, true);
        J.B = (int)b.B; J.stamp = place_stamp;
        st.nb_place = (int)((b.B + STAGE_THREADS * PLACE_EPT - 1) / (STAGE_THREADS * PLACE_EPT));
        if (sweep_period > 0) {
            const SweepSlice sw = slice_of(place_step);
            const long long n_pairs = ((long long)sw.n_u + 1) / 2 + ((long long)sw.n_i + 1) / 2;
            if (n_pairs <= SWEEP_ORDER_MAX) {
                J.n_pairs = (int)n_pairs;
                J.sw_tmp = w.sw_tmp; J.sw_order = w.sw_order;
                st.nb_sb = (int)((n_pairs + STAGE_BLOCK - 1) / STAGE_BLOCK);
            }
        }
    }
    return FR_OK;
}

extern "C" size_t fr_focf_row_words(int64_t n_users, int64_t n_items) { return 3 * ((size_t)n_users + (size_t)n_items); }

extern "C" int fr_focf_stage(const fr_table* U, const fr_table* I, const fr_focf_batch* claim, int32_t claim_stamp,
                             int32_t claim_gen, const fr_focf_batch* place, int32_t place_stamp, int32_t place_gen,
                             int32_t sweep_period, uint64_t* row_words, uint32_t* err_flag, void* stream_) {
    int rc;
    if ((rc = check_table(U, "fr_focf_stage(U)")) || (rc = check_table(I, "fr_focf_stage(I)"))) return rc;
    FR_CHECK_ARG(U->dim == I->dim && (claim || place), "fr_focf_stage: nothing to do");
    StageArgs st;
    if ((rc = make_stages(st, U, I, claim, claim_stamp, claim_gen, place, place_stamp, place_gen, sweep_period, row_words,
                          err_flag, place ? U->step + 1 : U->step, U->step)))
        return rc;
    const int nb = st.nb_claim + st.nb_sa + st.nb_place + st.nb_sb;
    ProfScope prof(K_FOCF_STAGE, (hipStream_t)stream_);
    FR_LAUNCH(prof, focf_stage_kernel, dim3(nb), dim3(STAGE_THREADS), 0, (hipStream_t)stream_, st);
    FR_CHECK_LAUNCH();
    return FR_OK;
}

static int focf_step_impl(const fr_table* U, const fr_table* I, const fr_adam* adam, const float* sst, int64_t B,
                          int32_t objective, float fair_weight, int32_t sweep_period, int32_t stamp, void* ws,
                          size_t ws_bytes, void* prev_ws, int64_t prev_B, float* prev_loss_out, float* loss_acc,
                          uint32_t* err_flag, void* stream_, const StageArgs* stages, uint64_t* row_words, int32_t gen) {
    hipStream_t stream = (hipStream_t)stream_;
    const bool staged = row_words != nullptr;
    int rc;
    if ((rc = check_table(U, "fr_focf_step(U)")) || (rc = check_table(I, "fr_focf_step(I)"))) return rc;
    FR_CHECK_ARG(U->dim == I->dim, "fr_focf_step: user dim %d != item dim %d", U->dim, I->dim);
    FR_CHECK_ARG(ws, "fr_focf_step: null pointer");
    FR_CHECK_ARG(objective >= FR_FOCF_NONE && objective <= FR_FOCF_OVER,
                 "fr_focf_step: objective %d needs batch-wide statistics before the update (use fr_focf_forward)", objective);
    FR_CHECK_ARG(objective == FR_FOCF_NONE || sst, "fr_focf_step: sst column required for a fairness objective");
    FR_CHECK_ARG(B >= 1 && B <= FR_SORT_MAX, "fr_focf_step: batch size %lld not in 1..%d", (long long)B, FR_SORT_MAX);
    FR_CHECK_ARG(U->step >= 1 && U->step == I->step, "fr_focf_step: table.step must be the step being applied (>=1), "
                 "the same for both tables");
    FR_CHECK_ARG(!U->step_dev && !I->step_dev, "fr_focf_step: device step counters are not supported");
    StepArgs a{};
    const FocfWs w = focf_layout(ws, B, U->dim);
    FR_CHECK_ARG(ws_bytes >= w.bytes, "fr_focf_step: workspace %zu < %zu bytes", ws_bytes, w.bytes);
    a.Up = U->p; a.Um = U->m; a.Uv = U->v; a.Ulast = U->last; a.Ustamp = U->stamp;
    a.Ip = I->p; a.Im = I->m; a.Iv = I->v; a.Ilast = I->last; a.Istamp = I->stamp;
    a.D = U->dim;
    a.step = U->step;
    a.c = make_adamc(adam);
    a.B = (int)B;
    a.objective = objective;
    a.fair_weight = fair_weight;
    a.task_rec = w.task_rec;
    a.task_info = w.task_info;
    static const int lead_pct = getenv("FAIRREC_STEP_LEAD") ? atoi(getenv("FAIRREC_STEP_LEAD")) : 100;

    a.hdr = w.nseg_i;
    a.mse_e = w.mse_e;
    a.term = w.term;
    a.ws = ws;
    a.err = err_flag;
    long long sweep_waves = 0;
    if (sweep_period > 0) {
        const SweepSlice sw = make_sweep_slice(U, I, sweep_period);
        a.lo_u = sw.lo_u; a.lo_i = sw.lo_i; a.n_u = sw.n_u; a.n_i = sw.n_i;
        a.skip_from = stamp;
        sweep_waves = ((long long)a.n_u + 1) / 2 + ((long long)a.n_i + 1) / 2;
        a.sw_order = sweep_waves <= SWEEP_ORDER_MAX ? w.sw_order : nullptr;
    }
    a.prev = prev_of(prev_ws, prev_B, U->dim, objective, fair_weight, prev_loss_out, loss_acc, staged);
    StageArgs st{};
    if (staged) {
        a.hcu = words_of(row_words, gen, U, I, false);
        a.hci = words_of(row_words, gen, U, I, true);
        if (stages) st = *stages;
    }
    {
        ProfScope prof(K_FOCF_STEP, stream);
        const long long per_wave = step_pairs((U->dim + 63) / 64) ? 2 : 1;
        const long long inter_blocks = ((B + per_wave - 1) / per_wave + STEP_WPB - 1) / STEP_WPB;
        const long long sweep_wg = (sweep_waves + STEP_WPB - 1) / STEP_WPB;
        const unsigned blocks = (unsigned)(1 + st.nb_claim + st.nb_sa + st.nb_place + st.nb_sb + sweep_wg + inter_blocks);
        a.lead = (int)(inter_blocks * lead_pct / 100);
        const dim3 block(64 * STEP_WPB);
        const int n_stage = st.nb_claim + st.nb_sa + st.nb_place + st.nb_sb;
#define STEP_PRE a.task_rec, a.sw_order, a.B, a.lead, a.n_u, a.n_i, n_stage, 0
        if (staged) {
            if (U->dim % 64 == 0) {
                FR_DISPATCH_E(U->dim, FR_LAUNCH(prof, (focf_step_kernel<E, true, true>), dim3(blocks), block, 0, stream, STEP_PRE, a, st));
            } else {
                FR_DISPATCH_E(U->dim, FR_LAUNCH(prof, (focf_step_kernel<E, false, true>), dim3(blocks), block, 0, stream, STEP_PRE, a, st));
            }
        } else if (U->dim % 64 == 0) {
            FR_DISPATCH_E(U->dim, FR_LAUNCH(prof, (focf_step_kernel<E, true, false>), dim3(blocks), block, 0, stream, STEP_PRE, a, st));
        } else {
            FR_DISPATCH_E(U->dim, FR_LAUNCH(prof, (focf_step_kernel<E, false, false>), dim3(blocks), block, 0, stream, STEP_PRE, a, st));
        }
#undef STEP_PRE
    }
    FR_CHECK_LAUNCH();
    return FR_OK;
}

extern "C" int fr_focf_step(const fr_table* U, const fr_table* I, const fr_adam* adam, const int64_t* user,
                            const int64_t* item, const float* rating, const float* sst, int64_t B, int32_t objective,
                            float fair_weight, int32_t sweep_period, int32_t stamp, void* ws, size_t ws_bytes,
                            float* loss_out, void* prev_ws, int64_t prev_B, float* prev_loss_out, float* loss_acc,
                            uint32_t* err_flag, void* stream_) {
    if (const int rc_ = check_focf_adam(adam, "fr_focf_step")) return rc_;
    (void)user; (void)item; (void)rating;
    (void)loss_out;
    return focf_step_impl(U, I, adam, sst, B, objective, fair_weight, sweep_period, stamp, ws, ws_bytes, prev_ws, prev_B,
                          prev_loss_out, loss_acc, err_flag, stream_, nullptr, nullptr, 0);
}

extern "C" int fr_focf_step_staged(const fr_table* U, const fr_table* I, const fr_adam* adam, const float* sst, int64_t B,
                                   int32_t objective, float fair_weight, int32_t sweep_period, int32_t stamp, int32_t gen,
                                   void* ws, size_t ws_bytes, void* prev_ws, int64_t prev_B, float* prev_loss_out,
                                   float* loss_acc, uint64_t* row_words, const fr_focf_batch* claim, int32_t claim_stamp,
                                   int32_t claim_gen, const fr_focf_batch* place, int32_t place_stamp, int32_t place_gen,
                                   uint32_t* err_flag, void* stream_) {
    if (const int rc_ = check_focf_adam(adam, "fr_focf_step_staged")) return rc_;
    FR_CHECK_ARG(row_words && gen >= 0 && gen < 3, "fr_focf_step_staged: row words / generation");
    FR_CHECK_ARG((!claim || claim_gen != gen) && (!place || place_gen != gen) && (!claim || !place || claim_gen != place_gen),
                 "fr_focf_step_staged: the three batches in flight need three different generations of row words");
    StageArgs st{};
    if (claim || place) {
        int rc;
        if ((rc = check_table(U, "fr_focf_step_staged(U)")) || (rc = check_table(I, "fr_focf_step_staged(I)"))) return rc;
        if ((rc = make_stages(st, U, I, claim, claim_stamp, claim_gen, place, place_stamp, place_gen, sweep_period, row_words,
                              err_flag, U->step + 2, U->step + 1)))
            return rc;
    }
    return focf_step_impl(U, I, adam, sst, B, objective, fair_weight, sweep_period, stamp, ws, ws_bytes, prev_ws, prev_B,
                          prev_loss_out, loss_acc, err_flag, stream_, &st, row_words, gen);
}

extern "C" int fr_focf_steps_many(const fr_table* U, const fr_table* I, const fr_adam* adam, const fr_focf_batch* batches,
                                  int32_t n, int32_t objective, float fair_weight, int32_t sweep_period, int32_t first_stamp,
                                  int32_t first_gen, void* prev_ws, int64_t prev_B, float* prev_loss_out, float* loss_ring,
                                  int32_t loss_slots, int32_t first_slot, float* loss_acc, uint64_t* row_words,
                                  uint32_t* err_flag, void* stream_) {
    if (const int rc_ = check_focf_adam(adam, "fr_focf_steps_many")) return rc_;
    FR_CHECK_ARG(U && I && batches && n >= 1, "fr_focf_steps_many: null pointer / no batch");
    FR_CHECK_ARG(loss_ring && loss_slots >= 1 && first_slot >= 0 && first_slot < loss_slots,
                 "fr_focf_steps_many: loss ring (float[4 * loss_slots]) and a first slot inside it");
    FR_CHECK_ARG(first_stamp >= 1 && first_stamp <= INT32_MAX - n && first_gen >= 0 && first_gen < 3,
                 "fr_focf_steps_many: first stamp / generation");
    FR_CHECK_ARG(U->step >= 1 && U->step == I->step && U->step <= INT32_MAX - n,
                 "fr_focf_steps_many: table.step must be the step the FIRST batch is applied at (>= 1), the same for both tables");
    for (int k = 0; k < n; ++k) {
        FR_CHECK_ARG(batches[k].ws && batches[k].user && batches[k].item && batches[k].rating,
                     "fr_focf_steps_many: batch %d: null pointer", k);
        for (int j = k + 1; j < n && j <= k + 3; ++j)
            FR_CHECK_ARG(batches[j].ws != batches[k].ws, "fr_focf_steps_many: batches %d and %d share a workspace", k, j);
        FR_CHECK_ARG(k > 2 || batches[k].ws != prev_ws,
                     "fr_focf_steps_many: batch %d uses the workspace whose loss is still to be reduced", k);
    }
    auto gen_of = [&](int k) { return (first_gen + k) % 3; };
    int rc;
    if ((rc = fr_focf_stage(U, I, &batches[0], first_stamp, gen_of(0), nullptr, 0, 0, sweep_period, row_words, err_flag, stream_)))
        return rc;
    if ((rc = fr_focf_stage(U, I, n > 1 ? &batches[1] : nullptr, first_stamp + 1, gen_of(1), &batches[0], first_stamp, gen_of(0),
                            sweep_period, row_words, err_flag, stream_)))
        return rc;
    fr_table tu = *U, ti = *I;
    for (int k = 0; k < n; ++k) {
        const fr_focf_batch& b = batches[k];
        const fr_focf_batch* place = k + 1 < n ? &batches[k + 1] : nullptr;
        const fr_focf_batch* claim = k + 2 < n ? &batches[k + 2] : nullptr;
        rc = fr_focf_step_staged(&tu, &ti, adam, b.sst, b.B, objective, fair_weight, sweep_period, first_stamp + k, gen_of(k),
                                 b.ws, b.ws_bytes, prev_ws, prev_B, prev_loss_out, loss_acc, row_words, claim,
                                 first_stamp + k + 2, gen_of(k + 2), place, first_stamp + k + 1, gen_of(k + 1), err_flag, stream_);
        if (rc) return rc;
        prev_ws = b.ws; prev_B = b.B;
        prev_loss_out = loss_ring + 4 * (size_t)((first_slot + k) % loss_slots);
        ++tu.step; ++ti.step;
    }
    return FR_OK;
}

#ifdef FR_LPT_STAMPS
extern "C" __attribute__((visibility("default"))) int fr_debug_lpt_stamps(unsigned long long* host_out) {
    FR_CHECK_HIP(hipDeviceSynchronize());
    FR_CHECK_HIP(hipMemcpyFromSymbol(host_out, HIP_SYMBOL(g_lpt_stamps), sizeof(unsigned long long) * 8));
    return FR_OK;
}
#endif

#if FR_STEP_TRACE
extern "C" __attribute__((visibility("default"))) int fr_debug_set_trace_step(int step) {
    FR_CHECK_HIP(hipMemcpyToSymbol(HIP_SYMBOL(g_trace_step), &step, sizeof(int)));
    return FR_OK;
}
extern "C" __attribute__((visibility("default"))) int fr_debug_step_trace(unsigned long long* host_out, int n_waves) {
    FR_CHECK_HIP(hipDeviceSynchronize());
    FR_CHECK_HIP(hipMemcpyFromSymbol(host_out, HIP_SYMBOL(g_step_trace), (size_t)n_waves * 32));
    FR_CHECK_HIP(hipMemcpyFromSymbol(host_out + 4 * (size_t)n_waves, HIP_SYMBOL(g_step_trace), (size_t)n_waves * 32,
                                     (size_t)65536 * 32));
    return FR_OK;
}
#endif

extern "C" int fr_focf_step_finish(void* ws, size_t ws_bytes, int64_t B, int32_t dim, int32_t objective,
                                   float fair_weight, float* loss_out, float* loss_acc, void* stream_) {
    FR_CHECK_ARG(ws && loss_out && B >= 1 && B <= FR_SORT_MAX && dim >= 1, "fr_focf_step_finish: bad argument");
    FR_CHECK_ARG(ws_bytes >= focf_layout(nullptr, B, dim).bytes, "fr_focf_step_finish: workspace too small");
    const PrevLoss pl = prev_of(ws, B, dim, objective, fair_weight, loss_out, loss_acc);
    hipLaunchKernelGGL(focf_step_finish_kernel, dim3(1), dim3(256), 0, (hipStream_t)stream_, pl);
    FR_CHECK_LAUNCH();
    return FR_OK;
}

extern "C" int fr_focf_step_finish_staged(void* ws, size_t ws_bytes, int64_t B, int32_t dim, int32_t objective,
                                          float fair_weight, float* loss_out, float* loss_acc, void* stream_) {
    FR_CHECK_ARG(ws && loss_out && B >= 1 && B <= FR_SORT_MAX && dim >= 1, "fr_focf_step_finish_staged: bad argument");
    FR_CHECK_ARG(ws_bytes >= focf_layout(nullptr, B, dim).bytes, "fr_focf_step_finish_staged: workspace too small");
    const PrevLoss pl = prev_of(ws, B, dim, objective, fair_weight, loss_out, loss_acc, true);
    hipLaunchKernelGGL(focf_step_finish_kernel, dim3(1), dim3(256), 0, (hipStream_t)stream_, pl);
    FR_CHECK_LAUNCH();
    return FR_OK;
}
```

Baseline: 290.0 million interactions/s.

## Fuse two consecutive FOCF steps into one paired kernel with cross-step row ordering

Adds a paired-step path that runs two consecutive batches in one launch. Rows shared between the two batches are tagged via mate row-word generations, ID flag bits packed into the row ids, and ordered write-through stores followed by a last-step stamp, so the second step can wait on rows the first step updates. Staging for four batches ahead is merged into a dual-stage kernel, and row-word generations go from 3 to 6. The aim is to halve launch and pipeline-drain overhead per step. The cost is spin-wait dependencies between the paired steps, extra ordering drains, and more complex scheduling.

After: 287.4 million interactions/s. No clear change (-0.9%).

```diff
diff --git a/recbole-fairrec_amd/csrc/focf_step.hip b/recbole-fairrec_amd/csrc/focf_step.hip
--- a/recbole-fairrec_amd/csrc/focf_step.hip
+++ b/recbole-fairrec_amd/csrc/focf_step.hip
@@ -76,6 +76,16 @@
 }
 __device__ __forceinline__ void drain_stores() { asm volatile("s_waitcnt vmcnt(0)" ::: "memory"); }
 
+constexpr unsigned ID_PREV = 0x80000000u, ID_NEXT = 0x40000000u;
+constexpr int ID_MASK = 0x3fffffff;
+constexpr int ROW_WORD_GENS = 6;
+constexpr int PAIR_WAIT_SPINS = 1 << 18;
+
+__device__ __forceinline__ void acquire_agent() { asm volatile("buffer_inv sc1\n\ts_waitcnt vmcnt(0)" ::: "memory"); }
+__device__ __forceinline__ int ld_sc1_gint(const int32_t* p) {
+    return __hip_atomic_load((const __attribute__((address_space(1))) int32_t*)p, __ATOMIC_RELAXED, __HIP_MEMORY_SCOPE_AGENT);
+}
+
 typedef __attribute__((address_space(1))) float gfloat;
 typedef __attribute__((address_space(1))) int32_t gint;
 __device__ __forceinline__ const gfloat* gp(const float* p) { return (const gfloat*)p; }
@@ -118,6 +128,18 @@
 }
 
 template <int E, bool FULL>
+__device__ __forceinline__ void ldrow_sc1(RowFrag<E>& f, const float* base, int D, int lane) {
+    const gfloat* g = gp(base);
+#pragma unroll
+    for (int e = 0; e < E; ++e) {
+        const int d = lane + 64 * e;
+        float val = (FULL || d < D) ? __hip_atomic_load(g + d, __ATOMIC_RELAXED, __HIP_MEMORY_SCOPE_AGENT) : 0.f;
+        asm volatile("" : "+v"(val));
+        f.x[e] = val;
+    }
+}
+
+template <int E, bool FULL>
 __device__ __forceinline__ void store_row_sc1(const RowFrag<E>& f, float* base, int D, int lane) {
     gfloat* g = gp(base);
 #pragma unroll
@@ -135,24 +157,28 @@
 #ifndef FR_WORD_STORE
 #define FR_WORD_STORE 1
 #endif
+template <bool CH = false>
 __device__ __forceinline__ void store_word(int32_t* p, int v) {
-#if FR_TROW_STORE == 1 && FR_WORD_STORE
-    __hip_atomic_store((gint*)p, v, __ATOMIC_RELAXED, __HIP_MEMORY_SCOPE_AGENT);
-#else
-    *(gint*)p = v;
-#endif
-}
+    if constexpr (CH || (FR_TROW_STORE == 1 && FR_WORD_STORE)) __hip_atomic_store((gint*)p, v, __ATOMIC_RELAXED, __HIP_MEMORY_SCOPE_AGENT);
+    else *(gint*)p = v;
+}
+template <bool CH = false>
 __device__ __forceinline__ void store_word(float* p, float v) {
-#if FR_TROW_STORE == 1 && FR_WORD_STORE
-    st_sc1g((gfloat*)p, v);
-#else
-    *(gfloat*)p = v;
-#endif
-}
-
-template <int E, bool FULL, bool WT = true>
+    if constexpr (CH || (FR_TROW_STORE == 1 && FR_WORD_STORE)) st_sc1g((gfloat*)p, v);
+    else *(gfloat*)p = v;
+}
+
+template <int E, bool FULL, bool WT = true, bool CH = false>
 __device__ __forceinline__ void store_trow(const RowFrag<E>& f, float* base, int D, int lane) {
     gfloat* g = gp(base);
+    if constexpr (CH) {
+#pragma unroll
+        for (int e = 0; e < E; ++e) {
+            const int d = lane + 64 * e;
+            if (FULL || d < D) { float val = f.x[e]; asm volatile("" : "+v"(val)); st_sc1g(g + d, val); }
+        }
+        return;
+    }
 #pragma unroll
     for (int e = 0; e < E; ++e) {
         const int d = lane + 64 * e;
@@ -209,6 +235,9 @@
     int32_t *Ulast, *Ustamp, *Ilast, *Istamp;
     int n_rows_u, n_rows_i, cap;
     uint32_t* err;
+    const unsigned long long *mate_u, *mate_i;
+    int mate_stamp;
+    unsigned mate_flag;
 };
 constexpr int STAGE_THREADS = 64 * STEP_WPB;
 
@@ -392,6 +421,7 @@
         f[e] = J.info[bc];
     }
     int nu[EPT], ni[EPT], k[EPT], key[EPT];
+    unsigned fu[EPT], fi[EPT];
     {
         unsigned long long wu[EPT], wi[EPT];
         int lu[EPT], li[EPT];
@@ -401,6 +431,11 @@
             wi[e] = J.hci[rec[e].y];
             lu[e] = s.Ulast[rec[e].x];
             li[e] = s.Ilast[rec[e].y];
+            fu[e] = fi[e] = 0u;
+            if (s.mate_u) {
+                fu[e] = (s.mate_u[rec[e].x] >> HC_TAG_SHIFT) == (unsigned long long)s.mate_stamp ? s.mate_flag : 0u;
+                fi[e] = (s.mate_i[rec[e].y] >> HC_TAG_SHIFT) == (unsigned long long)s.mate_stamp ? s.mate_flag : 0u;
+            }
         }
         const int cap = s.cap > 0 ? s.cap : 1024;
 #pragma unroll
@@ -415,11 +450,16 @@
                 const int base = atomicAdd(J.cp + 12, ni[e]);
                 __hip_atomic_fetch_add(J.hci + rec[e].y, (unsigned long long)base, __ATOMIC_RELAXED, __HIP_MEMORY_SCOPE_AGENT);
             }
-            k[e] = !ok[e] ? -1 : ((nu[e] > 1 || ni[e] > 1) && FR_LPT_SHARED_FIRST ? 0 : 1);
+            const bool shared = (nu[e] > 1 || ni[e] > 1) && FR_LPT_SHARED_FIRST;
+            k[e] = !ok[e] ? -1 : (shared ? 0 : 1);
             int cu = J.stamp - 1 - lu[e], ci = J.stamp - 1 - li[e];
             cu = cu < 0 ? 0 : (cu > cap ? cap : cu);
             ci = ci < 0 ? 0 : (ci > cap ? cap : ci);
             key[e] = 7 * (cu > ci ? cu : ci) + 2 * (cu > ci ? ci : cu);
+            if (s.mate_flag == ID_PREV && ok[e]) {
+                k[e] = ((fu[e] | fi[e]) & ID_PREV) ? 1 : 0;
+                if (shared && k[e] == 0) key[e] += 1 << 20;
+            }
         }
     }
     int before[EPT];
@@ -445,9 +485,9 @@
     for (int e = 0; e < EPT; ++e) {
         if (!ok[e]) continue;
         const int pos = k[e] == 0 ? base0 + before[e] : J.B - 1 - (base1 + (n1 - 1 - before[e]));
-        J.task_rec[pos] = rec[e];
+        J.task_rec[pos] = make_int4((int)((unsigned)rec[e].x | fu[e]), (int)((unsigned)rec[e].y | fi[e]), rec[e].z, rec[e].w);
         J.task_info[pos] = make_int4(f[e].x | nu[e] << 16, f[e].y | ni[e] << 16, 0, b[e]);
-        J.info[b[e]] = make_int4(f[e].x, f[e].y, nu[e], ni[e]);
+        J.info[b[e]] = make_int4(f[e].x, f[e].y, (int)((unsigned)nu[e] | fu[e]), (int)((unsigned)ni[e] | fi[e]));
     }
     if (sb == 0 && threadIdx.x == 0) {
         const unsigned e1 = (unsigned)J.cp[9], e2 = (unsigned)J.cp[10];
@@ -551,12 +591,22 @@
     return true;
 }
 
-template <int E, bool FULL>
+template <int E, bool FULL, bool CH = false>
 __device__ __forceinline__ void adam_write(float* Tp, float* Tm, float* Tv, int32_t* Tlast, int D, int step,
                                            const AdamC& c, int row, RowFrag<E>& p, RowFrag<E>& m, RowFrag<E>& v,
-                                           const RowFrag<E>& g, float2 s, int lane) {
+                                           const RowFrag<E>& g, float2 s, int lane, bool ordered = false) {
 #pragma unroll
     for (int e = 0; e < E; ++e) adam_elem(p.x[e], m.x[e], v.x[e], g.x[e], s.x, s.y, c);
+    if constexpr (CH) {
+        if (ordered) {
+            store_trow<E, FULL, false, true>(p, Tp + (size_t)row * D, D, lane);
+            store_trow<E, FULL, false, true>(m, Tm + (size_t)row * D, D, lane);
+            store_trow<E, FULL, false, true>(v, Tv + (size_t)row * D, D, lane);
+            drain_stores();
+            if (lane == 0) store_word<true>(Tlast + row, step);
+            return;
+        }
+    }
     store_trow<E, FULL, false>(p, Tp + (size_t)row * D, D, lane);
     store_trow<E, FULL, false>(m, Tm + (size_t)row * D, D, lane);
     store_trow<E, FULL, false>(v, Tv + (size_t)row * D, D, lane);
@@ -652,9 +702,9 @@
     adam_write<E, FULL>(KA(Up), KA(Um), KA(Uv), KA(Ulast), D, KA(step), c, ur, p, m, v, g, s, lane);
 }
 
-template <int E, bool FULL>
+template <int E, bool FULL, bool CH = false>
 __device__ __forceinline__ void user_finish_c(KV kv, const AdamC& c, const FocfWs& w, int ur, int base, int nu, float2 s,
-                                              int lane) {
+                                              int lane, bool ordered = false) {
     const int D = FULL ? 64 * E : KA(D);
     const Members mem = load_members(w.perm_u, w.seg_start_u, base, nu, lane);
     const int c0 = __builtin_amdgcn_readlane(members_chunk(mem, 0, lane), 0);
@@ -663,14 +713,14 @@
     load_row_sc1<E, FULL>(m, w.side[1] + (size_t)c0 * D, D, lane);
     load_row_sc1<E, FULL>(v, w.side[2] + (size_t)c0 * D, D, lane);
     handed_grad_sum<E, FULL>(g, nu, [&](int jb) { return members_chunk(mem, jb, lane); }, w.coef, w.side[3], D, lane);
-    adam_write<E, FULL>(KA(Up), KA(Um), KA(Uv), KA(Ulast), D, KA(step), c, ur, p, m, v, g, s, lane);
-}
-
-template <int E, bool FULL, bool CLAIM>
+    adam_write<E, FULL, CH>(KA(Up), KA(Um), KA(Uv), KA(Ulast), D, KA(step), c, ur, p, m, v, g, s, lane, ordered);
+}
+
+template <int E, bool FULL, bool CLAIM, bool CH = false>
 __device__ __forceinline__ void step_shared_rows(KV kv, const AdamC& c, int b, int lane, int ur, int ir, int iux, int iix,
                                                  int seg_u, int seg_i, float dot, float coef, float smin, float smax,
                                                  float K, RowFrag<E>& pu, RowFrag<E>& mu, RowFrag<E>& vu, RowFrag<E>& pi,
-                                                 RowFrag<E>& mi, RowFrag<E>& vi) {
+                                                 RowFrag<E>& mi, RowFrag<E>& vi, bool ord_u = false, bool ord_i = false) {
     const int D = FULL ? 64 * E : KA(D);
     const bool fair = KA(objective) != FR_FOCF_NONE;
     const int nu = iux >> 16, ni = iix >> 16, j0u = iux & 0xffff, j0i = iix & 0xffff;
@@ -697,12 +747,12 @@
         RowFrag<E> gi;
 #pragma unroll
         for (int e = 0; e < E; ++e) gi.x[e] = coef * pu.x[e];
-        adam_write<E, FULL>(KA(Ip), KA(Im), KA(Iv), KA(Ilast), D, KA(step), c, ir, pi, mi, vi, gi, s, lane);
+        adam_write<E, FULL, CH>(KA(Ip), KA(Im), KA(Iv), KA(Ilast), D, KA(step), c, ir, pi, mi, vi, gi, s, lane, ord_i);
         if (lane == 0) st_sc1(w.coef + b, coef);
         drain_stores();
         if constexpr (CLAIM) {
             const unsigned long long old = hc_arrive(KA(hcu) + ur, lane);
-            if (hc_cnt(old) == 1) user_finish_c<E, FULL>(kv, c, w, ur, hc_base(old), nu, s, lane);
+            if (hc_cnt(old) == 1) user_finish_c<E, FULL, CH>(kv, c, w, ur, hc_base(old), nu, s, lane, ord_u);
         } else {
             if (arrive_last(w.cnt_u + seg_u, nu, lane)) user_finish<E, FULL>(kv, c, w, j0u, nu, s, lane);
         }
@@ -725,8 +775,9 @@
     const bool big = ni > 64;
     int my_b = 0, my_u = 0, my_iux = 0, my_seg = 0;
     float my_pr = 0.f, my_rt = 0.f, my_s = 0.f;
+    int my_ord = 0;
     auto load_chunk = [&](int jb) {
-        my_b = 0; my_u = 0; my_iux = 0; my_seg = 0;
+        my_b = 0; my_u = 0; my_iux = 0; my_seg = 0; my_ord = 0;
         my_pr = 0.f; my_rt = 0.f; my_s = 0.f;
         int mb = 0;
         if constexpr (CLAIM) mb = members_chunk(mem, jb, lane);
@@ -738,7 +789,8 @@
             my_pr = ld_sc1(w.pred + my_b);
             my_u = rq.x; my_rt = __int_as_float(rq.z); my_s = __int_as_float(rq.w);
             if constexpr (CLAIM) {
-                my_iux = fq.z << 16;
+                my_iux = (int)((unsigned)fq.z << 16);
+                if constexpr (CH) my_ord = ((unsigned)fq.z & ID_NEXT) ? 1 : 0;
             } else {
                 my_iux = fq.x; my_seg = fq.y;
             }
@@ -826,12 +878,13 @@
                     RowFrag<E> gu;
 #pragma unroll
                     for (int e = 0; e < E; ++e) gu.x[e] = cq[q] * pi.x[e];
-                    adam_write<E, FULL>(KA(Up), KA(Um), KA(Uv), KA(Ulast), D, KA(step), c, uq[q], p[q], m[q], v[q], gu, s, lane);
+                    adam_write<E, FULL, CH>(KA(Up), KA(Um), KA(Uv), KA(Ulast), D, KA(step), c, uq[q], p[q], m[q], v[q], gu, s, lane,
+                                            CH && __builtin_amdgcn_readlane(my_ord, t0 + q < cnt ? t0 + q : cnt - 1) != 0);
                 }
             }
         }
     }
-    adam_write<E, FULL>(KA(Ip), KA(Im), KA(Iv), KA(Ilast), D, KA(step), c, ir, pi, mi, vi, gi, s, lane);
+    adam_write<E, FULL, CH>(KA(Ip), KA(Im), KA(Iv), KA(Ilast), D, KA(step), c, ir, pi, mi, vi, gi, s, lane, ord_i);
     if (!shared_users) return;
     drain_stores();
     for (int jb = 0; jb < ni; jb += 64) {
@@ -845,7 +898,9 @@
             if constexpr (CLAIM) {
                 const int uu = __builtin_amdgcn_readlane(my_u, t);
                 const unsigned long long old = hc_arrive(KA(hcu) + uu, lane);
-                if (hc_cnt(old) == 1) user_finish_c<E, FULL>(kv, c, w, uu, hc_base(old), iq >> 16, s, lane);
+                if (hc_cnt(old) == 1)
+                    user_finish_c<E, FULL, CH>(kv, c, w, uu, hc_base(old), iq >> 16, s, lane,
+                                               CH && __builtin_amdgcn_readlane(my_ord, t) != 0);
             } else {
                 const int sg = __builtin_amdgcn_readlane(my_seg, t);
                 if (arrive_last(w.cnt_u + sg, iq >> 16, lane)) user_finish<E, FULL>(kv, c, w, iq & 0xffff, iq >> 16, s, lane);
@@ -876,13 +931,15 @@
     g = in0 ? dx * q / cc : -dx * q / cc;
 }
 
-template <int E, bool FULL, bool CLAIM>
+template <int E, bool FULL, bool CLAIM, bool CH = false>
 __device__ __forceinline__ void step_finish(KV kv, const AdamC& c, int lane, int q, RowFrag<E>& pu, RowFrag<E>& mu,
                                             RowFrag<E>& vu, RowFrag<E>& pi, RowFrag<E>& mi, RowFrag<E>& vi) {
     const int D = FULL ? 64 * E : KA(D);
     const bool fair = KA(objective) != FR_FOCF_NONE;
     const int4 vrec = KA(task_rec)[q], vinf = KA(task_info)[q], vhd = *reinterpret_cast<const int4*>(KA(hdr));
-    const int4 rec = make_int4(uniform(vrec.x), uniform(vrec.y), uniform(vrec.z), uniform(vrec.w));
+    constexpr int IDM = CH ? ID_MASK : -1;
+    const int4 rec = make_int4(uniform(vrec.x) & IDM, uniform(vrec.y) & IDM, uniform(vrec.z), uniform(vrec.w));
+    const bool ord_u = CH && ((unsigned)uniform(vrec.x) & ID_NEXT), ord_i = CH && ((unsigned)uniform(vrec.y) & ID_NEXT);
     const int4 inf = make_int4(uniform(vinf.x), uniform(vinf.y), uniform(vinf.z), uniform(vinf.w));
     const int4 hd = make_int4(uniform(vhd.x), 0, uniform(vhd.z), uniform(vhd.w));
     const int ur = rec.x, ir = rec.y;
@@ -921,6 +978,20 @@
             mu.x[e] = M.x; mi.x[e] = M.y;
             vu.x[e] = V.x; vi.x[e] = V.y;
         }
+        if (CH && (ord_u || ord_i)) {
+            store_trow<E, FULL, true, true>(pu, KA(Up) + (size_t)ur * D, D, lane);
+            store_trow<E, FULL, true, true>(mu, KA(Um) + (size_t)ur * D, D, lane);
+            store_trow<E, FULL, true, true>(vu, KA(Uv) + (size_t)ur * D, D, lane);
+            store_trow<E, FULL, true, true>(pi, KA(Ip) + (size_t)ir * D, D, lane);
+            store_trow<E, FULL, true, true>(mi, KA(Im) + (size_t)ir * D, D, lane);
+            store_trow<E, FULL, true, true>(vi, KA(Iv) + (size_t)ir * D, D, lane);
+            drain_stores();
+            if (lane == 0) {
+                store_word<true>(KA(Ulast) + ur, KA(step));
+                store_word<true>(KA(Ilast) + ir, KA(step));
+            }
+            return;
+        }
         store_trow<E, FULL>(pu, KA(Up) + (size_t)ur * D, D, lane);
         store_trow<E, FULL>(mu, KA(Um) + (size_t)ur * D, D, lane);
         store_trow<E, FULL>(vu, KA(Uv) + (size_t)ur * D, D, lane);
@@ -933,11 +1004,11 @@
         }
         return;
     }
-    step_shared_rows<E, FULL, CLAIM>(kv, c, b, lane, ur, ir, iux, iix, seg_u, seg_i, dot, coef, smin, smax, K, pu, mu, vu, pi, mi,
-                                     vi);
-}
-
-template <int E, bool FULL>
+    step_shared_rows<E, FULL, CLAIM, CH>(kv, c, b, lane, ur, ir, iux, iix, seg_u, seg_i, dot, coef, smin, smax, K, pu, mu, vu, pi, mi,
+                                         vi, ord_u, ord_i);
+}
+
+template <int E, bool FULL, bool ORDERED = false>
 __device__ __forceinline__ void adam_store_both(KV kv, const AdamC& c, int lane, int ur, int ir, float coef, float2 sc,
                                                 RowFrag<E> pu, RowFrag<E> mu, RowFrag<E> vu, RowFrag<E> pi,
                                                 RowFrag<E> mi, RowFrag<E> vi) {
@@ -955,19 +1026,21 @@
         mu.x[e] = M.x; mi.x[e] = M.y;
         vu.x[e] = V.x; vi.x[e] = V.y;
     }
-    store_trow<E, FULL>(pu, KA(Up) + (size_t)ur * D, D, lane);
-    store_trow<E, FULL>(mu, KA(Um) + (size_t)ur * D, D, lane);
-    store_trow<E, FULL>(vu, KA(Uv) + (size_t)ur * D, D, lane);
-    store_trow<E, FULL>(pi, KA(Ip) + (size_t)ir * D, D, lane);
-    store_trow<E, FULL>(mi, KA(Im) + (size_t)ir * D, D, lane);
-    store_trow<E, FULL>(vi, KA(Iv) + (size_t)ir * D, D, lane);
-    if (lane == 0) {
-        store_word(KA(Ulast) + ur, KA(step));
-        store_word(KA(Ilast) + ir, KA(step));
-    }
-}
-
-template <int E, bool FULL, bool CLAIM>
+    store_trow<E, FULL, true, ORDERED>(pu, KA(Up) + (size_t)ur * D, D, lane);
+    store_trow<E, FULL, true, ORDERED>(mu, KA(Um) + (size_t)ur * D, D, lane);
+    store_trow<E, FULL, true, ORDERED>(vu, KA(Uv) + (size_t)ur * D, D, lane);
+    store_trow<E, FULL, true, ORDERED>(pi, KA(Ip) + (size_t)ir * D, D, lane);
+    store_trow<E, FULL, true, ORDERED>(mi, KA(Im) + (size_t)ir * D, D, lane);
+    store_trow<E, FULL, true, ORDERED>(vi, KA(Iv) + (size_t)ir * D, D, lane);
+    if constexpr (!ORDERED) {
+        if (lane == 0) {
+            store_word(KA(Ulast) + ur, KA(step));
+            store_word(KA(Ilast) + ir, KA(step));
+        }
+    }
+}
+
+template <int E, bool FULL, bool CLAIM, bool CH = false>
 __device__ __forceinline__ void step_finish_pair(KV kv, const AdamC& c, int lane, int q, int q1, bool has1, TwoRows<E> us,
                                                  TwoRows<E> is) {
     const int obj = KA(objective);
@@ -1013,7 +1086,11 @@
     }
     const float coef0 = __builtin_bit_cast(float, __builtin_amdgcn_readlane(__builtin_bit_cast(int, coef), 0));
     const float coef1 = __builtin_bit_cast(float, __builtin_amdgcn_readlane(__builtin_bit_cast(int, coef), 1));
-    const int ur0 = uniform(vr0.x), ir0 = uniform(vr0.y), ur1 = uniform(vr1.x), ir1 = uniform(vr1.y);
+    constexpr int IDM = CH ? ID_MASK : -1;
+    const int fu0 = uniform(vr0.x), fi0 = uniform(vr0.y), fu1 = uniform(vr1.x), fi1 = uniform(vr1.y);
+    const int ur0 = fu0 & IDM, ir0 = fi0 & IDM, ur1 = fu1 & IDM, ir1 = fi1 & IDM;
+    const bool ou0 = CH && ((unsigned)fu0 & ID_NEXT), oi0 = CH && ((unsigned)fi0 & ID_NEXT);
+    const bool ou1 = CH && ((unsigned)fu1 & ID_NEXT), oi1 = CH && ((unsigned)fi1 & ID_NEXT);
     const int iux0 = uniform(vi0.x), iix0 = uniform(vi0.y), iux1 = uniform(vi1.x), iix1 = uniform(vi1.y);
     const bool un0 = (iux0 >> 16) == 1 && (iix0 >> 16) == 1;
     const bool un1 = has1 && (iux1 >> 16) == 1 && (iix1 >> 16) == 1;
@@ -1021,12 +1098,37 @@
     if (un0 && un1) {
         RowFrag<E> a0 = us.pA, a1 = us.mA, a2 = us.vA, a3 = is.pA, a4 = is.mA, a5 = is.vA;
         RowFrag<E> b0 = us.pB, b1 = us.mB, b2 = us.vB, b3 = is.pB, b4 = is.mB, b5 = is.vB;
-        adam_store_both<E, FULL>(kv, c, lane, ur0, ir0, coef0, sc, a0, a1, a2, a3, a4, a5);
-        adam_store_both<E, FULL>(kv, c, lane, ur1, ir1, coef1, sc, b0, b1, b2, b3, b4, b5);
+        if (CH && (ou0 || oi0 || ou1 || oi1)) {
+            adam_store_both<E, FULL, true>(kv, c, lane, ur0, ir0, coef0, sc, a0, a1, a2, a3, a4, a5);
+            adam_store_both<E, FULL, true>(kv, c, lane, ur1, ir1, coef1, sc, b0, b1, b2, b3, b4, b5);
+            drain_stores();
+            if (lane == 0) {
+                store_word<true>(KA(Ulast) + ur0, KA(step));
+                store_word<true>(KA(Ilast) + ir0, KA(step));
+                store_word<true>(KA(Ulast) + ur1, KA(step));
+                store_word<true>(KA(Ilast) + ir1, KA(step));
+            }
+        } else {
+            adam_store_both<E, FULL>(kv, c, lane, ur0, ir0, coef0, sc, a0, a1, a2, a3, a4, a5);
+            adam_store_both<E, FULL>(kv, c, lane, ur1, ir1, coef1, sc, b0, b1, b2, b3, b4, b5);
+        }
         return;
     }
-    if (un0) adam_store_both<E, FULL>(kv, c, lane, ur0, ir0, coef0, sc, us.pA, us.mA, us.vA, is.pA, is.mA, is.vA);
-    if (un1) adam_store_both<E, FULL>(kv, c, lane, ur1, ir1, coef1, sc, us.pB, us.mB, us.vB, is.pB, is.mB, is.vB);
+    auto both = [&](int ur, int ir, float coef, bool ordered, const RowFrag<E>& p0, const RowFrag<E>& p1, const RowFrag<E>& p2,
+                    const RowFrag<E>& p3, const RowFrag<E>& p4, const RowFrag<E>& p5) {
+        if (CH && ordered) {
+            adam_store_both<E, FULL, true>(kv, c, lane, ur, ir, coef, sc, p0, p1, p2, p3, p4, p5);
+            drain_stores();
+            if (lane == 0) {
+                store_word<true>(KA(Ulast) + ur, KA(step));
+                store_word<true>(KA(Ilast) + ir, KA(step));
+            }
+        } else {
+            adam_store_both<E, FULL>(kv, c, lane, ur, ir, coef, sc, p0, p1, p2, p3, p4, p5);
+        }
+    };
+    if (un0) both(ur0, ir0, coef0, ou0 || oi0, us.pA, us.mA, us.vA, is.pA, is.mA, is.vA);
+    if (un1) both(ur1, ir1, coef1, ou1 || oi1, us.pB, us.mB, us.vB, is.pB, is.mB, is.vB);
     if (un0 && (un1 || !has1)) return;
     for (int k = 0; k < (has1 ? 2 : 1); ++k) {
         if (k) {
@@ -1038,9 +1140,9 @@
         }
         if (!(k ? un1 : un0)) {
             const int sg = uniform(k ? vi1.z : vi0.z);
-            step_shared_rows<E, FULL, CLAIM>(kv, c, uniform(k ? vi1.w : vi0.w), lane, k ? ur1 : ur0, k ? ir1 : ir0, k ? iux1 : iux0,
+            step_shared_rows<E, FULL, CLAIM, CH>(kv, c, uniform(k ? vi1.w : vi0.w), lane, k ? ur1 : ur0, k ? ir1 : ir0, k ? iux1 : iux0,
                                       k ? iix1 : iix0, sg & 0xffff, sg >> 16, k ? d1 : d0, k ? coef1 : coef0, smin, smax, K,
-                                      us.pA, us.mA, us.vA, is.pA, is.mA, is.vA);
+                                      us.pA, us.mA, us.vA, is.pA, is.mA, is.vA, k ? ou1 : ou0, k ? oi1 : oi0);
         }
     }
 }
@@ -1048,7 +1150,17 @@
 #if FR_STEP_TRACE
 #define g_phase phase_stamps
 #endif
-template <int E, bool FULL, bool PAIR, bool CLAIM>
+__device__ __forceinline__ void await_published(const int32_t* Tlast, int row, int want, uint32_t* err, int lane) {
+    int t = 0;
+    for (int spin = 0; spin < PAIR_WAIT_SPINS; ++spin) {
+        t = ld_sc1_gint(Tlast + row);
+        if (t >= want) break;
+        __builtin_amdgcn_s_sleep(8);
+    }
+    if (uniform(t) < want && lane == 0 && err) atomicOr(err, FR_DEV_ERR_PIPE_WAIT);
+}
+
+template <int E, bool FULL, bool PAIR, bool CLAIM, bool CH = false>
 __device__ __forceinline__ void step_task(KV kv, bool sweeper, int q, int n_pairs, int lane, const int4* rec0,
                                           const int32_t* order0, int B0
 #if FR_STEP_TRACE
@@ -1064,7 +1176,7 @@
     int tA, tB;
     if (sweeper) {
         if (const int32_t* so = order0) {
-            const int oq = so[q], on = so[n_pairs];
+            const int oq = gp(so)[q], on = gp(so)[n_pairs];
             q = uniform(on) == n_pairs ? uniform(oq) : q;
         }
         const int pairs_u = (KA(n_u) + 1) >> 1;
@@ -1109,26 +1221,51 @@
         const bool has1 = q + 1 < B0;
         const int q1 = has1 ? q + 1 : q;
         const int4 vrec0 = gp(rec0)[q], vrec1 = gp(rec0)[q1];
-        const int u0 = uniform(vrec0.x), i0 = uniform(vrec0.y), u1 = uniform(vrec1.x), i1 = uniform(vrec1.y);
+        const int fu0 = uniform(vrec0.x), fi0 = uniform(vrec0.y), fu1 = uniform(vrec1.x), fi1 = uniform(vrec1.y);
+        const int u0 = CH ? fu0 & ID_MASK : fu0, i0 = CH ? fi0 & ID_MASK : fi0;
+        const int u1 = CH ? fu1 & ID_MASK : fu1, i1 = CH ? fi1 & ID_MASK : fi1;
 #if FR_STEP_TRACE
         g_phase[2] = __builtin_amdgcn_s_memrealtime();
 #endif
-        const int lu0 = gp((const int32_t*)KA(Ulast))[u0], lu1 = gp((const int32_t*)KA(Ulast))[u1];
-        const int li0 = gp((const int32_t*)KA(Ilast))[i0], li1 = gp((const int32_t*)KA(Ilast))[i1];
+        const int upto = KA(step) - 1;
         TwoRows<E> it;
-        ldrow<E, FULL>(r.pA, KA(Up) + (size_t)u0 * D, D, lane);
-        ldrow<E, FULL>(r.pB, KA(Up) + (size_t)u1 * D, D, lane);
-        ldrow<E, FULL>(it.pA, KA(Ip) + (size_t)i0 * D, D, lane);
-        ldrow<E, FULL>(it.pB, KA(Ip) + (size_t)i1 * D, D, lane);
-        ldrow<E, FULL>(r.mA, KA(Um) + (size_t)u0 * D, D, lane);
-        ldrow<E, FULL>(r.vA, KA(Uv) + (size_t)u0 * D, D, lane);
-        ldrow<E, FULL>(r.mB, KA(Um) + (size_t)u1 * D, D, lane);
-        ldrow<E, FULL>(r.vB, KA(Uv) + (size_t)u1 * D, D, lane);
-        ldrow<E, FULL>(it.mA, KA(Im) + (size_t)i0 * D, D, lane);
-        ldrow<E, FULL>(it.vA, KA(Iv) + (size_t)i0 * D, D, lane);
-        ldrow<E, FULL>(it.mB, KA(Im) + (size_t)i1 * D, D, lane);
-        ldrow<E, FULL>(it.vB, KA(Iv) + (size_t)i1 * D, D, lane);
-        const int upto = KA(step) - 1;
+        int lu0, lu1, li0, li1;
+        if (CH && (fu0 | fi0 | fu1 | fi1) < 0) {
+            if (fu0 < 0) await_published(KA(Ulast), u0, upto, KA(err), lane);
+            if (fu1 < 0) await_published(KA(Ulast), u1, upto, KA(err), lane);
+            if (fi0 < 0) await_published(KA(Ilast), i0, upto, KA(err), lane);
+            if (fi1 < 0) await_published(KA(Ilast), i1, upto, KA(err), lane);
+            acquire_agent();
+            lu0 = ld_sc1_gint(KA(Ulast) + u0); lu1 = ld_sc1_gint(KA(Ulast) + u1);
+            li0 = ld_sc1_gint(KA(Ilast) + i0); li1 = ld_sc1_gint(KA(Ilast) + i1);
+            ldrow_sc1<E, FULL>(r.pA, KA(Up) + (size_t)u0 * D, D, lane);
+            ldrow_sc1<E, FULL>(r.pB, KA(Up) + (size_t)u1 * D, D, lane);
+            ldrow_sc1<E, FULL>(it.pA, KA(Ip) + (size_t)i0 * D, D, lane);
+            ldrow_sc1<E, FULL>(it.pB, KA(Ip) + (size_t)i1 * D, D, lane);
+            ldrow_sc1<E, FULL>(r.mA, KA(Um) + (size_t)u0 * D, D, lane);
+            ldrow_sc1<E, FULL>(r.vA, KA(Uv) + (size_t)u0 * D, D, lane);
+            ldrow_sc1<E, FULL>(r.mB, KA(Um) + (size_t)u1 * D, D, lane);
+            ldrow_sc1<E, FULL>(r.vB, KA(Uv) + (size_t)u1 * D, D, lane);
+            ldrow_sc1<E, FULL>(it.mA, KA(Im) + (size_t)i0 * D, D, lane);
+            ldrow_sc1<E, FULL>(it.vA, KA(Iv) + (size_t)i0 * D, D, lane);
+            ldrow_sc1<E, FULL>(it.mB, KA(Im) + (size_t)i1 * D, D, lane);
+            ldrow_sc1<E, FULL>(it.vB, KA(Iv) + (size_t)i1 * D, D, lane);
+        } else {
+            lu0 = gp((const int32_t*)KA(Ulast))[u0]; lu1 = gp((const int32_t*)KA(Ulast))[u1];
+            li0 = gp((const int32_t*)KA(Ilast))[i0]; li1 = gp((const int32_t*)KA(Ilast))[i1];
+            ldrow<E, FULL>(r.pA, KA(Up) + (size_t)u0 * D, D, lane);
+            ldrow<E, FULL>(r.pB, KA(Up) + (size_t)u1 * D, D, lane);
+            ldrow<E, FULL>(it.pA, KA(Ip) + (size_t)i0 * D, D, lane);
+            ldrow<E, FULL>(it.pB, KA(Ip) + (size_t)i1 * D, D, lane);
+            ldrow<E, FULL>(r.mA, KA(Um) + (size_t)u0 * D, D, lane);
+            ldrow<E, FULL>(r.vA, KA(Uv) + (size_t)u0 * D, D, lane);
+            ldrow<E, FULL>(r.mB, KA(Um) + (size_t)u1 * D, D, lane);
+            ldrow<E, FULL>(r.vB, KA(Uv) + (size_t)u1 * D, D, lane);
+            ldrow<E, FULL>(it.mA, KA(Im) + (size_t)i0 * D, D, lane);
+            ldrow<E, FULL>(it.vA, KA(Iv) + (size_t)i0 * D, D, lane);
+            ldrow<E, FULL>(it.mB, KA(Im) + (size_t)i1 * D, D, lane);
+            ldrow<E, FULL>(it.vB, KA(Iv) + (size_t)i1 * D, D, lane);
+        }
         const int tu0 = uniform(lu0), tu1 = uniform(lu1), ti0 = uniform(li0), ti1 = uniform(li1);
 #if FR_STEP_TRACE
         g_phase[0] = __builtin_amdgcn_s_memrealtime();
@@ -1139,22 +1276,37 @@
 #if FR_STEP_TRACE
         g_phase[1] = __builtin_amdgcn_s_memrealtime();
 #endif
-        step_finish_pair<E, FULL, CLAIM>(kv, c, lane, q, q1, has1, r, it);
+        step_finish_pair<E, FULL, CLAIM, CH>(kv, c, lane, q, q1, has1, r, it);
         return;
     }
     const int4 vrec = rec0[q];
-    const int ur = uniform(vrec.x), ir = uniform(vrec.y);
-    const int lu = KA(Ulast)[ur], li = KA(Ilast)[ir];
-    ldrow<E, FULL>(r.pA, KA(Up) + (size_t)ur * D, D, lane);
-    ldrow<E, FULL>(r.pB, KA(Ip) + (size_t)ir * D, D, lane);
-    ldrow<E, FULL>(r.mA, KA(Um) + (size_t)ur * D, D, lane);
-    ldrow<E, FULL>(r.vA, KA(Uv) + (size_t)ur * D, D, lane);
-    ldrow<E, FULL>(r.mB, KA(Im) + (size_t)ir * D, D, lane);
-    ldrow<E, FULL>(r.vB, KA(Iv) + (size_t)ir * D, D, lane);
+    const int fur = uniform(vrec.x), fir = uniform(vrec.y);
+    const int ur = CH ? fur & ID_MASK : fur, ir = CH ? fir & ID_MASK : fir;
+    int lu, li;
+    if (CH && (fur | fir) < 0) {
+        if (fur < 0) await_published(KA(Ulast), ur, KA(step) - 1, KA(err), lane);
+        if (fir < 0) await_published(KA(Ilast), ir, KA(step) - 1, KA(err), lane);
+        acquire_agent();
+        lu = ld_sc1_gint(KA(Ulast) + ur); li = ld_sc1_gint(KA(Ilast) + ir);
+        ldrow_sc1<E, FULL>(r.pA, KA(Up) + (size_t)ur * D, D, lane);
+        ldrow_sc1<E, FULL>(r.pB, KA(Ip) + (size_t)ir * D, D, lane);
+        ldrow_sc1<E, FULL>(r.mA, KA(Um) + (size_t)ur * D, D, lane);
+        ldrow_sc1<E, FULL>(r.vA, KA(Uv) + (size_t)ur * D, D, lane);
+        ldrow_sc1<E, FULL>(r.mB, KA(Im) + (size_t)ir * D, D, lane);
+        ldrow_sc1<E, FULL>(r.vB, KA(Iv) + (size_t)ir * D, D, lane);
+    } else {
+        lu = KA(Ulast)[ur]; li = KA(Ilast)[ir];
+        ldrow<E, FULL>(r.pA, KA(Up) + (size_t)ur * D, D, lane);
+        ldrow<E, FULL>(r.pB, KA(Ip) + (size_t)ir * D, D, lane);
+        ldrow<E, FULL>(r.mA, KA(Um) + (size_t)ur * D, D, lane);
+        ldrow<E, FULL>(r.vA, KA(Uv) + (size_t)ur * D, D, lane);
+        ldrow<E, FULL>(r.mB, KA(Im) + (size_t)ir * D, D, lane);
+        ldrow<E, FULL>(r.vB, KA(Iv) + (size_t)ir * D, D, lane);
+    }
     tA = uniform(lu);
     tB = uniform(li);
     replay_two<E>(r, tA, tB, KA(step) - 1, c, lane);
-    step_finish<E, FULL, CLAIM>(kv, c, lane, q, r.pA, r.mA, r.vA, r.pB, r.mB, r.vB);
+    step_finish<E, FULL, CLAIM, CH>(kv, c, lane, q, r.pA, r.mA, r.vA, r.pB, r.mB, r.vB);
 }
 
 __host__ __device__ constexpr bool step_pairs(int E) { return E <= 1; }
@@ -1240,9 +1392,60 @@
 #endif
 }
 
+template <int E, bool FULL>
+__global__ __launch_bounds__(64 * STEP_WPB, step_waves(E)) void focf_step_pair_kernel(const int4* pre_rec, const int32_t* pre_order,
+                                                                                      int pre_B, int pre_lead, int pre_nu, int pre_ni,
+                                                                                      int pre_stage, int pre_first, StepArgs a,
+                                                                                      StepArgs b, StageArgs s0, StageArgs s1,
+                                                                                      int n_stage0, PrevLoss prev2) {
+    const int lane = threadIdx.x & 63;
+    const int wib = uniform((int)(threadIdx.x >> 6));
+    const int stage0 = 1 + pre_lead;
+    const int bx = (int)blockIdx.x;
+    if (bx == 0) {
+        if (a.prev.loss_out) step_reduce_loss<64 * STEP_WPB>(a.prev);
+        if (prev2.loss_out) {
+            __syncthreads();
+            step_reduce_loss<64 * STEP_WPB>(prev2);
+        }
+    } else if (bx >= stage0 && bx < stage0 + pre_stage) {
+        const int sb = bx - stage0;
+        if (sb < n_stage0) stage_block(s0, sb);
+        else stage_block(s1, sb - n_stage0);
+    } else {
+        const bool second = bx >= pre_first;
+        static_assert(STEP_PRELOAD_DWORDS * 4 % alignof(StepArgs) == 0 && sizeof(StepArgs) % 4 == 0, "a and b follow the scalars");
+        const unsigned* kp = reinterpret_cast<const unsigned*>(
+            (const void*)(const __attribute__((address_space(4))) void*)__builtin_amdgcn_kernarg_segment_ptr());
+        const int off = STEP_PRELOAD_DWORDS + (second ? (int)(sizeof(StepArgs) / 4) : 0);
+        KV kv;
+        kv.v0 = kp[off + lane];
+        kv.v1 = lane < (int)(sizeof(StepArgs) / 4) - 64 ? kp[off + 64 + lane] : 0u;
+        const int4* rec0 = second ? b.task_rec : pre_rec;
+        const int32_t* order0 = second ? b.sw_order : pre_order;
+        const int B0 = second ? b.B : pre_B, lead = second ? b.lead : pre_lead;
+        const int nu = second ? b.n_u : pre_nu, ni = second ? b.n_i : pre_ni;
+        const int x = second ? bx - pre_first : bx - 1 - (bx >= stage0 ? pre_stage : 0);
+        const int n_pairs = ((nu + 1) >> 1) + ((ni + 1) >> 1);
+        constexpr bool PAIR = step_pairs(E);
+        const bool sweeper = x >= lead;
+        const int q = ((sweeper ? x - lead : x) * STEP_WPB + wib) * (!sweeper && PAIR ? 2 : 1);
+#if FR_STEP_TRACE
+        unsigned long long ph[4] = {0, 0, 0, 0};
+        if (q < (sweeper ? n_pairs : B0)) step_task<E, FULL, PAIR, true, true>(kv, sweeper, q, n_pairs, lane, rec0, order0, B0, ph);
+#else
+        if (q < (sweeper ? n_pairs : B0)) step_task<E, FULL, PAIR, true, true>(kv, sweeper, q, n_pairs, lane, rec0, order0, B0);
+#endif
+    }
+}
+
 __global__ __launch_bounds__(256) void focf_step_finish_kernel(PrevLoss pl) { step_reduce_loss<256>(pl); }
 
 __global__ __launch_bounds__(STAGE_THREADS) void focf_stage_kernel(StageArgs st) { stage_block(st, (int)blockIdx.x); }
+__global__ __launch_bounds__(STAGE_THREADS) void focf_stage2_kernel(StageArgs s0, StageArgs s1, int n_stage0) {
+    if ((int)blockIdx.x < n_stage0) stage_block(s0, (int)blockIdx.x);
+    else stage_block(s1, (int)blockIdx.x - n_stage0);
+}
 
 struct SwOrderJob {
     const int32_t *Ulast, *Ustamp, *Ilast, *Istamp;
@@ -1555,7 +1758,7 @@
     if (claim) {
         const fr_focf_batch& b = *claim;
         FR_CHECK_ARG(b.user && b.item && b.rating && b.ws && b.B >= 1 && b.B <= FR_SORT_MAX && claim_stamp >= 1 &&
-                         claim_gen >= 0 && claim_gen < 3, "fr_focf_stage: batch to claim");
+                         claim_gen >= 0 && claim_gen < ROW_WORD_GENS, "fr_focf_stage: batch to claim");
         const FocfWs w = focf_layout(b.ws, b.B, U->dim);
         FR_CHECK_ARG(b.ws_bytes >= w.bytes, "fr_focf_stage: workspace %zu < %zu bytes", b.ws_bytes, w.bytes);
         ClaimJob& J = st.c;
@@ -1577,7 +1780,7 @@
     }
     if (place) {
         const fr_focf_batch& b = *place;
-        FR_CHECK_ARG(b.ws && b.B >= 1 && b.B <= FR_SORT_MAX && place_stamp >= 1 && place_gen >= 0 && place_gen < 3,
+        FR_CHECK_ARG(b.ws && b.B >= 1 && b.B <= FR_SORT_MAX && place_stamp >= 1 && place_gen >= 0 && place_gen < ROW_WORD_GENS,
                      "fr_focf_stage: batch to place");
         const FocfWs w = focf_layout(b.ws, b.B, U->dim);
         FR_CHECK_ARG(b.ws_bytes >= w.bytes, "fr_focf_stage: workspace %zu < %zu bytes", b.ws_bytes, w.bytes);
@@ -1601,7 +1804,9 @@
     return FR_OK;
 }
 
-extern "C" size_t fr_focf_row_words(int64_t n_users, int64_t n_items) { return 3 * ((size_t)n_users + (size_t)n_items); }
+extern "C" size_t fr_focf_row_words(int64_t n_users, int64_t n_items) {
+    return (size_t)ROW_WORD_GENS * ((size_t)n_users + (size_t)n_items);
+}
 
 extern "C" int fr_focf_stage(const fr_table* U, const fr_table* I, const fr_focf_batch* claim, int32_t claim_stamp,
                              int32_t claim_gen, const fr_focf_batch* place, int32_t place_stamp, int32_t place_gen,
@@ -1620,12 +1825,10 @@
     return FR_OK;
 }
 
-static int focf_step_impl(const fr_table* U, const fr_table* I, const fr_adam* adam, const float* sst, int64_t B,
-                          int32_t objective, float fair_weight, int32_t sweep_period, int32_t stamp, void* ws,
-                          size_t ws_bytes, void* prev_ws, int64_t prev_B, float* prev_loss_out, float* loss_acc,
-                          uint32_t* err_flag, void* stream_, const StageArgs* stages, uint64_t* row_words, int32_t gen) {
-    hipStream_t stream = (hipStream_t)stream_;
-    const bool staged = row_words != nullptr;
+static int make_step_args(StepArgs& a, long long& sweep_waves, long long& inter_blocks, const fr_table* U, const fr_table* I,
+                          const fr_adam* adam, const float* sst, int64_t B, int32_t objective, float fair_weight,
+                          int32_t sweep_period, int32_t skip_from, void* ws, size_t ws_bytes, uint32_t* err_flag,
+                          uint64_t* row_words, int32_t gen) {
     int rc;
     if ((rc = check_table(U, "fr_focf_step(U)")) || (rc = check_table(I, "fr_focf_step(I)"))) return rc;
     FR_CHECK_ARG(U->dim == I->dim, "fr_focf_step: user dim %d != item dim %d", U->dim, I->dim);
@@ -1637,7 +1840,7 @@
     FR_CHECK_ARG(U->step >= 1 && U->step == I->step, "fr_focf_step: table.step must be the step being applied (>=1), "
                  "the same for both tables");
     FR_CHECK_ARG(!U->step_dev && !I->step_dev, "fr_focf_step: device step counters are not supported");
-    StepArgs a{};
+    a = StepArgs{};
     const FocfWs w = focf_layout(ws, B, U->dim);
     FR_CHECK_ARG(ws_bytes >= w.bytes, "fr_focf_step: workspace %zu < %zu bytes", ws_bytes, w.bytes);
     a.Up = U->p; a.Um = U->m; a.Uv = U->v; a.Ulast = U->last; a.Ustamp = U->stamp;
@@ -1657,28 +1860,42 @@
     a.term = w.term;
     a.ws = ws;
     a.err = err_flag;
-    long long sweep_waves = 0;
+    sweep_waves = 0;
     if (sweep_period > 0) {
         const SweepSlice sw = make_sweep_slice(U, I, sweep_period);
         a.lo_u = sw.lo_u; a.lo_i = sw.lo_i; a.n_u = sw.n_u; a.n_i = sw.n_i;
-        a.skip_from = stamp;
+        a.skip_from = skip_from;
         sweep_waves = ((long long)a.n_u + 1) / 2 + ((long long)a.n_i + 1) / 2;
         a.sw_order = sweep_waves <= SWEEP_ORDER_MAX ? w.sw_order : nullptr;
     }
+    if (row_words) {
+        a.hcu = words_of(row_words, gen, U, I, false);
+        a.hci = words_of(row_words, gen, U, I, true);
+    }
+    const long long per_wave = step_pairs((U->dim + 63) / 64) ? 2 : 1;
+    inter_blocks = ((B + per_wave - 1) / per_wave + STEP_WPB - 1) / STEP_WPB;
+    a.lead = (int)(inter_blocks * lead_pct / 100);
+    return FR_OK;
+}
+
+static int focf_step_impl(const fr_table* U, const fr_table* I, const fr_adam* adam, const float* sst, int64_t B,
+                          int32_t objective, float fair_weight, int32_t sweep_period, int32_t stamp, void* ws,
+                          size_t ws_bytes, void* prev_ws, int64_t prev_B, float* prev_loss_out, float* loss_acc,
+                          uint32_t* err_flag, void* stream_, const StageArgs* stages, uint64_t* row_words, int32_t gen) {
+    hipStream_t stream = (hipStream_t)stream_;
+    const bool staged = row_words != nullptr;
+    StepArgs a;
+    long long sweep_waves, inter_blocks;
+    if (const int rc = make_step_args(a, sweep_waves, inter_blocks, U, I, adam, sst, B, objective, fair_weight, sweep_period, stamp,
+                                      ws, ws_bytes, err_flag, row_words, gen))
+        return rc;
     a.prev = prev_of(prev_ws, prev_B, U->dim, objective, fair_weight, prev_loss_out, loss_acc, staged);
     StageArgs st{};
-    if (staged) {
-        a.hcu = words_of(row_words, gen, U, I, false);
-        a.hci = words_of(row_words, gen, U, I, true);
-        if (stages) st = *stages;
-    }
+    if (staged && stages) st = *stages;
     {
         ProfScope prof(K_FOCF_STEP, stream);
-        const long long per_wave = step_pairs((U->dim + 63) / 64) ? 2 : 1;
-        const long long inter_blocks = ((B + per_wave - 1) / per_wave + STEP_WPB - 1) / STEP_WPB;
         const long long sweep_wg = (sweep_waves + STEP_WPB - 1) / STEP_WPB;
         const unsigned blocks = (unsigned)(1 + st.nb_claim + st.nb_sa + st.nb_place + st.nb_sb + sweep_wg + inter_blocks);
-        a.lead = (int)(inter_blocks * lead_pct / 100);
         const dim3 block(64 * STEP_WPB);
         const int n_stage = st.nb_claim + st.nb_sa + st.nb_place + st.nb_sb;
 #define STEP_PRE a.task_rec, a.sw_order, a.B, a.lead, a.n_u, a.n_i, n_stage, 0
@@ -1718,7 +1935,7 @@
                                    int32_t claim_gen, const fr_focf_batch* place, int32_t place_stamp, int32_t place_gen,
                                    uint32_t* err_flag, void* stream_) {
     if (const int rc_ = check_focf_adam(adam, "fr_focf_step_staged")) return rc_;
-    FR_CHECK_ARG(row_words && gen >= 0 && gen < 3, "fr_focf_step_staged: row words / generation");
+    FR_CHECK_ARG(row_words && gen >= 0 && gen < ROW_WORD_GENS, "fr_focf_step_staged: row words / generation");
     FR_CHECK_ARG((!claim || claim_gen != gen) && (!place || place_gen != gen) && (!claim || !place || claim_gen != place_gen),
                  "fr_focf_step_staged: the three batches in flight need three different generations of row words");
     StageArgs st{};
@@ -1731,6 +1948,108 @@
     }
     return focf_step_impl(U, I, adam, sst, B, objective, fair_weight, sweep_period, stamp, ws, ws_bytes, prev_ws, prev_B,
                           prev_loss_out, loss_acc, err_flag, stream_, &st, row_words, gen);
+}
+
+static int focf_steps_paired(const fr_table* U, const fr_table* I, const fr_adam* adam, const fr_focf_batch* batches, int32_t n,
+                             int32_t objective, float fair_weight, int32_t sweep_period, int32_t first_stamp, int32_t first_gen,
+                             void* prev_ws, int64_t prev_B, float* prev_loss_out, float* loss_ring, int32_t loss_slots,
+                             int32_t first_slot, float* loss_acc, uint64_t* row_words, uint32_t* err_flag, void* stream_) {
+    hipStream_t stream = (hipStream_t)stream_;
+    int rc;
+    if ((rc = check_table(U, "fr_focf_steps_many(U)")) || (rc = check_table(I, "fr_focf_steps_many(I)"))) return rc;
+    FR_CHECK_ARG(U->dim == I->dim, "fr_focf_steps_many: user dim %d != item dim %d", U->dim, I->dim);
+    for (int k = 0; k < n; ++k) {
+        for (int j = k + 1; j < n && j <= k + 7; ++j)
+            FR_CHECK_ARG(batches[j].ws != batches[k].ws, "fr_focf_steps_many: batches %d and %d share a workspace", k, j);
+        FR_CHECK_ARG(k > 3 || batches[k].ws != prev_ws,
+                     "fr_focf_steps_many: batch %d uses the workspace whose loss is still to be reduced", k);
+    }
+    const int step0 = U->step;
+    const int n_pair = n / 2;
+    auto gen_of = [&](int k) { return (first_gen + k) % ROW_WORD_GENS; };
+    auto stamp_of = [&](int k) { return first_stamp + k; };
+    auto slot_of = [&](int k) { return loss_ring + 4 * (size_t)((first_slot + k) % loss_slots); };
+    auto nb_of = [](const StageArgs& st) { return st.nb_claim + st.nb_sa + st.nb_place + st.nb_sb; };
+    auto stages_of = [&](StageArgs& st, int kc, int kp) -> int {
+        const fr_focf_batch* claim = kc >= 0 && kc < n ? &batches[kc] : nullptr;
+        const fr_focf_batch* place = kp >= 0 && kp < n ? &batches[kp] : nullptr;
+        st = StageArgs{};
+        if (!claim && !place) return FR_OK;
+        const int rc2 = make_stages(st, U, I, claim, claim ? stamp_of(kc) : 0, claim ? gen_of(kc) : 0, place,
+                                    place ? stamp_of(kp) : 0, place ? gen_of(kp) : 0, sweep_period, row_words, err_flag,
+                                    step0 + kc, step0 + kp);
+        if (rc2) return rc2;
+        if (place && kp < 2 * n_pair) {
+            const int mate = kp ^ 1;
+            st.mate_u = words_of(row_words, gen_of(mate), U, I, false);
+            st.mate_i = words_of(row_words, gen_of(mate), U, I, true);
+            st.mate_stamp = stamp_of(mate);
+            st.mate_flag = (kp & 1) ? ID_PREV : ID_NEXT;
+        }
+        return FR_OK;
+    };
+    for (int q = 0; q < 2; ++q) {
+        StageArgs s0, s1;
+        if ((rc = stages_of(s0, 2 * q, 2 * q - 2)) || (rc = stages_of(s1, 2 * q + 1, 2 * q - 1))) return rc;
+        const int nb = nb_of(s0) + nb_of(s1);
+        if (!nb) continue;
+        ProfScope prof(K_FOCF_STAGE, stream);
+        FR_LAUNCH(prof, focf_stage2_kernel, dim3(nb), dim3(STAGE_THREADS), 0, stream, s0, s1, nb_of(s0));
+        FR_CHECK_LAUNCH();
+    }
+    fr_table tu = *U, ti = *I;
+    for (int j = 0; j < n_pair; ++j) {
+        const int ka = 2 * j, kb = ka + 1;
+        const fr_focf_batch &A = batches[ka], &Bb = batches[kb];
+        StepArgs a, b;
+        long long sw_a, sw_b, ib_a, ib_b;
+        tu.step = ti.step = step0 + ka;
+        if ((rc = make_step_args(a, sw_a, ib_a, &tu, &ti, adam, A.sst, A.B, objective, fair_weight, sweep_period, stamp_of(ka), A.ws,
+                                 A.ws_bytes, err_flag, row_words, gen_of(ka))))
+            return rc;
+        tu.step = ti.step = step0 + kb;
+        if ((rc = make_step_args(b, sw_b, ib_b, &tu, &ti, adam, Bb.sst, Bb.B, objective, fair_weight, sweep_period, stamp_of(ka),
+                                 Bb.ws, Bb.ws_bytes, err_flag, row_words, gen_of(kb))))
+            return rc;
+        a.lead = (int)ib_a;
+        b.lead = (int)ib_b;
+        PrevLoss prev2{};
+        if (j == 0) {
+            a.prev = prev_of(prev_ws, prev_B, U->dim, objective, fair_weight, prev_loss_out, loss_acc, true);
+        } else {
+            a.prev = prev_of(batches[ka - 2].ws, batches[ka - 2].B, U->dim, objective, fair_weight, slot_of(ka - 2), loss_acc, true);
+            prev2 = prev_of(batches[ka - 1].ws, batches[ka - 1].B, U->dim, objective, fair_weight, slot_of(ka - 1), loss_acc, true);
+        }
+        StageArgs s0, s1;
+        if ((rc = stages_of(s0, ka + 4, ka + 2)) || (rc = stages_of(s1, ka + 5, ka + 3))) return rc;
+        const int n_stage0 = nb_of(s0), n_stage = n_stage0 + nb_of(s1);
+        const long long wg_a = (sw_a + STEP_WPB - 1) / STEP_WPB, wg_b = (sw_b + STEP_WPB - 1) / STEP_WPB;
+        const long long first = 1 + ib_a + n_stage + wg_a;
+        const unsigned blocks = (unsigned)(first + ib_b + wg_b);
+        const dim3 block(64 * STEP_WPB);
+        ProfScope prof(K_FOCF_STEP, stream);
+#define PAIR_ARGS a.task_rec, a.sw_order, a.B, a.lead, a.n_u, a.n_i, n_stage, (int)first, a, b, s0, s1, n_stage0, prev2
+        if (U->dim % 64 == 0) {
+            FR_DISPATCH_E(U->dim, FR_LAUNCH(prof, (focf_step_pair_kernel<E, true>), dim3(blocks), block, 0, stream, PAIR_ARGS));
+        } else {
+            FR_DISPATCH_E(U->dim, FR_LAUNCH(prof, (focf_step_pair_kernel<E, false>), dim3(blocks), block, 0, stream, PAIR_ARGS));
+        }
+#undef PAIR_ARGS
+        FR_CHECK_LAUNCH();
+    }
+    const int kl = 2 * n_pair - 2;
+    if ((rc = fr_focf_step_finish_staged(batches[kl].ws, batches[kl].ws_bytes, batches[kl].B, U->dim, objective, fair_weight,
+                                         slot_of(kl), loss_acc, stream_)))
+        return rc;
+    if (n & 1) {
+        const fr_focf_batch& L = batches[n - 1];
+        tu.step = ti.step = step0 + n - 1;
+        const StageArgs none{};
+        return focf_step_impl(&tu, &ti, adam, L.sst, L.B, objective, fair_weight, sweep_period, stamp_of(n - 1), L.ws, L.ws_bytes,
+                              batches[n - 2].ws, batches[n - 2].B, slot_of(n - 2), loss_acc, err_flag, stream_, &none, row_words,
+                              gen_of(n - 1));
+    }
+    return FR_OK;
 }
 
 extern "C" int fr_focf_steps_many(const fr_table* U, const fr_table* I, const fr_adam* adam, const fr_focf_batch* batches,
@@ -1754,6 +2073,10 @@
         FR_CHECK_ARG(k > 2 || batches[k].ws != prev_ws,
                      "fr_focf_steps_many: batch %d uses the workspace whose loss is still to be reduced", k);
     }
+    static const bool pair_env = !(getenv("FAIRREC_FOCF_PAIR") && atoi(getenv("FAIRREC_FOCF_PAIR")) == 0);
+    if (pair_env && n >= 2 && sweep_period != 1 && U->n_rows <= ID_MASK && I->n_rows <= ID_MASK && row_words)
+        return focf_steps_paired(U, I, adam, batches, n, objective, fair_weight, sweep_period, first_stamp, first_gen, prev_ws,
+                                 prev_B, prev_loss_out, loss_ring, loss_slots, first_slot, loss_acc, row_words, err_flag, stream_);
     auto gen_of = [&](int k) { return (first_gen + k) % 3; };
     int rc;
     if ((rc = fr_focf_stage(U, I, &batches[0], first_stamp, gen_of(0), nullptr, 0, 0, sweep_period, row_words, err_flag, stream_)))
```
